# yewsiang/Transferable3D

Measured on AMD Instinct MI355X. Metric: frustums/sec fwd+bwd, higher is better.
Workload: dtype f32

## Files before the change

include/t3d.h:

```cpp
#ifndef T3D_H_
#define T3D_H_

#include <stdint.h>

#ifdef __cplusplus
extern "C" {
#endif

#define T3D_OK 0
#define T3D_ERR_ARG (-1)
#define T3D_ERR_SHAPE (-2)
#define T3D_ERR_LAUNCH (-3)
#define T3D_ERR_ABI (-4)

#define T3D_ABI_VERSION 3
#define T3D_V2_SIZE_pointmlp_fwd_args 200
#define T3D_V2_SIZE_pointmlp_dgrad_args 168
#define T3D_V2_SIZE_pointmlp_wgrad_args 144
#define T3D_V2_SIZE_pointmlp_dgrad_gram_args 168
#define T3D_V2_SIZE_pointmlp_gram_args 96
#define T3D_V2_SIZE_seg_head_args 208
#define T3D_V2_SIZE_boxpc_rep_args 104

#define T3D_TILE_ROWS 128
// ... 159 lines not shown
typedef struct {
  const float* psum_dz;
  const float* psum_y;
  const float* coef;
  int B, N, tiles_per_frustum, rows_per_frustum;
  float alpha;
  float* out;
} t3d_dy_colsum_args;
int t3d_dy_colsum(const t3d_dy_colsum_args* args, t3d_stream_t stream);

typedef struct {
  const float* w;
  const float* bias;
  const float* coef;
  int K, N;
  float* p_slabs;
  float* rc_slabs;
  float* wc;
} t3d_pool_bwd_prep_args;
int t3d_pool_bwd_prep(const t3d_pool_bwd_prep_args* args, t3d_stream_t stream);

typedef struct {
  const int32_t* argidx;
  const float* dpool;
  const float* wc;
  int B, N, K;
  int rows_per_frustum;
  float* s;
  int32_t* row_live;
} t3d_pool_sparse_rows_args;
int t3d_pool_sparse_rows(const t3d_pool_sparse_rows_args* args, t3d_stream_t stream);

typedef struct {
  uint32_t struct_size;
  t3d_act_src a;
  const float* p;
  const float* rowconst;
  const float* add_in;
  const int32_t* add_live;
  const float* prev_y;
  const float* prev_scale;
  const float* prev_shift;
  float* out;
  float* psum_dz;
  float* psum_dzy;
  int M, K;
  int rows_per_frustum;
  int dtype;
  int arith;
} t3d_pointmlp_dgrad_gram_args;
int t3d_pointmlp_dgrad_gram(const t3d_pointmlp_dgrad_gram_args* args, t3d_stream_t stream);

typedef struct {
  uint32_t struct_size;
  t3d_act_src a;
  float* slabs;
  int M, K;
  int rows_per_frustum;
  int rows_per_split;
  int arith;
} t3d_pointmlp_gram_args;
int t3d_pointmlp_gram(const t3d_pointmlp_gram_args* args, t3d_stream_t stream);

int t3d_gram_plan(int M, int K, int dtype, int* rows_per_split, int* one_pass);

typedef struct {
  t3d_act_src a;
  int M, K;
  int rows_per_frustum;
  float* part;
} t3d_act_colsum_args;
int t3d_act_colsum(const t3d_act_colsum_args* args, t3d_stream_t stream);

typedef struct {
  t3d_act_src a;
  const int32_t* argidx;
  const float* dpool;
  const float* coef;
  const float* w;
  const float* bias;
  const float* g;
  const float* abar;
  int B, K, N;
  int rows_per_frustum;
  float* dw;
} t3d_pool_wgrad_finish_args;
int t3d_pool_wgrad_finish(const t3d_pool_wgrad_finish_args* args, t3d_stream_t stream);

int t3d_pool_bwd_stage1(const t3d_pointmlp_gram_args* gram, const t3d_act_colsum_args* colsum,
                        const t3d_pool_bwd_prep_args* prep, t3d_stream_t stream);
int t3d_pool_bwd_stage2(const t3d_pool_wgrad_finish_args* finish, const t3d_pointmlp_dgrad_gram_args* dgrad,
                        t3d_stream_t stream);

typedef struct {
  const float* in;  int ld_in;  int K;
  const float* in2; int ld_in2; int K2;
  const float* w;
  const float* bias;
  const float* gamma; const float* beta;
  float* moving_mean; float* moving_var;
  const float* decay;
  float eps; int is_training; int unbiased_ema;
  int act; float leaky_alpha;
  const float* drop_mask; float keep_prob;
  const float* add_in; int ld_add; int add_n;
  float* y;
  float* out; int ld_out;
  float* mean; float* invstd;
  int B, N;
} t3d_fc_fwd_args;
int t3d_fc_fwd(const t3d_fc_fwd_args* args, t3d_stream_t stream);

typedef struct {
  const float* dout; int ld_dout;
  const float* dy_next; const float* w_next; int N_next;
  const float* in;  int ld_in;  int K;
  const float* in2; int ld_in2; int K2;
  const float* y; const float* out; int ld_out;
  const float* gamma; const float* beta; const float* mean; const float* invstd;
  int bn_training;
  int act; float leaky_alpha;
  const float* drop_mask; float keep_prob;
  float* dy;
  float* dw; float* dbias; float* dgamma; float* dbeta;
  int B, N;
// ... 410 lines not shown
  float bn_init_decay, bn_decay_rate, bn_decay_step, bn_decay_clip;
  float beta1, beta2;
  int batch_size;
  int step_offset;
} t3d_schedule;
int t3d_schedule_step(float* hyper, const t3d_schedule* s, t3d_stream_t stream);

int t3d_adam_tf_step(float* params, const float* grads, float* m, float* v, int64_t n,
                     const float* hyper, float beta1, float beta2, float eps, float grad_scale,
                     t3d_stream_t stream);

typedef struct { int64_t off; int64_t n; int32_t blk0; int32_t reserved; } t3d_adam_range;
int t3d_reduce_slabs_adam(const float* slab_base, float* grad_base, const t3d_slab_desc* table_dev, int n_tensors, int max_numel,
                          float* params, float* m, float* v, const t3d_adam_range* ranges_dev, int n_ranges, int n_range_blocks,
                          const float* hyper, float beta1, float beta2, float eps, float grad_scale, t3d_stream_t stream);

int t3d_split_x3(const float* src, void* planes, int64_t n, int64_t plane_stride, t3d_stream_t stream);

typedef struct {
  int64_t off;
  int32_t K, N;
  int32_t fwd, dgrad;
  int32_t blk0;
  int32_t reserved;
} t3d_x3_frag_entry;
int t3d_split_x3_frag(const float* params, void* planes_fwd, void* planes_dgrad, int64_t plane_stride, const t3d_x3_frag_entry* table,
                      int n_entries, int n_blocks, t3d_stream_t stream);

int t3d_step_head_takes(const t3d_pointmlp_fwd_args* fwd);
int t3d_step_head(const t3d_pointmlp_fwd_args* fwd, const float* params, void* planes_fwd, void* planes_dgrad, int64_t plane_stride,
                  const t3d_x3_frag_entry* table, int n_entries, int n_blocks, float* hyper, const t3d_schedule* sched,
                  t3d_stream_t stream);

int t3d_momentum_step(float* params, const float* grads, float* accum, int64_t n, const float* hyper, float momentum,
                      float grad_scale, t3d_stream_t stream);

typedef struct {
  t3d_act_src a;
  const float* mask;
  float keep_prob;
  float* out;
  int M, K;
  int rows_per_frustum;
} t3d_act_dropout_args;
int t3d_act_dropout(const t3d_act_dropout_args* args, t3d_stream_t stream);

int t3d_cast_bf16(const float* src, void* dst, int64_t n, t3d_stream_t stream);

int t3d_dropout_mask(float* mask, int64_t n, float keep_prob, uint32_t seed, const float* hyper,
                     t3d_stream_t stream);

enum { T3D_SMALL_BN_BWD_FINALIZE = 1, T3D_SMALL_FC_BWD = 2, T3D_SMALL_FC_DINPUT = 3, T3D_SMALL_DY_COLSUM = 4,
       T3D_SMALL_BN_FWD_FINALIZE = 5, T3D_SMALL_FC_FWD = 6, T3D_SMALL_POOL_BWD_MID = 7 };
typedef struct {
  const float* slab_base;
  float* grad_base;
  const t3d_slab_desc* table_dev;
  int n_tensors, max_numel;
  t3d_pool_sparse_rows_args sparse;
} t3d_pool_bwd_mid_args;
typedef struct {
  int kind;
  int depends;
  union {
    t3d_bn_bwd_finalize_args bn_bwd;
    t3d_fc_bwd_args fc_bwd;
    t3d_fc_dinput_args fc_dinput;
    t3d_dy_colsum_args dy_colsum;
    t3d_bn_fwd_finalize_args bn_fwd;
    t3d_fc_fwd_args fc_fwd;
    t3d_pool_bwd_mid_args mid;
  } u;
} t3d_small_op;
int t3d_small_pair(const t3d_small_op* a, const t3d_small_op* b, t3d_stream_t stream);

#define T3D_RIDER_MAX_OPS 10
typedef struct {
  t3d_small_op ops[T3D_RIDER_MAX_OPS];
  int n_ops;
  int n_wg;
  int lds_bytes;
  unsigned* sync;
} t3d_rider_set;
int t3d_riders_plan(t3d_rider_set* riders);
int t3d_run_riders(const t3d_rider_set* riders, t3d_stream_t stream);
int t3d_pointmlp_fwd_r(const t3d_pointmlp_fwd_args* args, const t3d_rider_set* riders, t3d_stream_t stream);
int t3d_pointmlp_wgrad_r(const t3d_pointmlp_wgrad_args* args, const t3d_rider_set* riders, t3d_stream_t stream);
int t3d_pointmlp_bwd_r(const t3d_pointmlp_dgrad_args* dgrad, const t3d_pointmlp_wgrad_args* wgrad, const t3d_rider_set* riders,
                       t3d_stream_t stream);
int t3d_pool_bwd_stage1_r(const t3d_pointmlp_gram_args* gram, const t3d_act_colsum_args* colsum, const t3d_pool_bwd_prep_args* prep,
                          const t3d_rider_set* riders, t3d_stream_t stream);
int t3d_pool_bwd_stage2_r(const t3d_pool_wgrad_finish_args* finish, const t3d_pointmlp_dgrad_gram_args* dgrad,
                          const t3d_rider_set* riders, t3d_stream_t stream);
int t3d_pointmlp_fwd_hosts_riders(const t3d_pointmlp_fwd_args* args);
int t3d_pointmlp_wgrad_hosts_riders(const t3d_pointmlp_wgrad_args* args);
int t3d_pointmlp_bwd_hosts_riders(const t3d_pointmlp_dgrad_args* dgrad, const t3d_pointmlp_wgrad_args* wgrad);
int t3d_pool_bwd_stage1_hosts_riders(const t3d_pointmlp_gram_args* gram, const t3d_act_colsum_args* colsum, const t3d_pool_bwd_prep_args* prep);
int t3d_pool_bwd_stage2_hosts_riders(const t3d_pool_wgrad_finish_args* finish, const t3d_pointmlp_dgrad_gram_args* dgrad);

typedef struct {
  uint32_t struct_size;
  const double* points;
  const int64_t* scene_offsets;
  const double* rtilt;
  const double* K;
  const int32_t* scene_jobs;
  int n_scenes; int max_scene_points; int C_src; int C; int n_jobs; int num_points;
  const double* box2d;
  int perturb_box2d;
  const double* perturb_draws;
  const double* box3d;
  const int32_t* job_key;
  uint32_t seed;
  const int32_t* choice;
  const int64_t* mask_offsets;
  uint64_t* masks;
  int32_t* seg_prefix;
  double* box2d_out;
  double* frustum_angle;
  int32_t* n_in_box;
  int32_t* count;
  int32_t* index;
  double* out_points;
  int32_t* label;
} t3d_frustum_extract_args;
#define T3D_V2_SIZE_frustum_extract_args 208
// ... 183 lines not shown
```

transferable3d_amd/abi.py:

```python
import ctypes as C
import os

F = C.POINTER(C.c_float)
I = C.POINTER(C.c_int32)
D = C.POINTER(C.c_double)
L = C.POINTER(C.c_int64)
i32, f32 = C.c_int, C.c_float

TILE_ROWS = 128
F32, BF16 = 0, 1
DTYPE_BY_NAME = {'f32': F32, 'bf16': BF16}
ARITH_AUTO, ARITH_FP32_MFMA, ARITH_BF16X3, ARITH_BF16 = 0, 1, 2, 3
ARITH_BY_NAME = {'auto': ARITH_AUTO, 'fp32_mfma': ARITH_FP32_MFMA, 'bf16x3': ARITH_BF16X3}
ARITH_NAMES = {ARITH_FP32_MFMA: 'fp32_mfma', ARITH_BF16X3: 'bf16x3', ARITH_BF16: 'bf16'}
ABI_VERSION = 3
ERR_ABI = -4
ACT_NONE, ACT_RELU, ACT_LEAKY_RELU, ACT_TANH = 0, 1, 2, 3
ACT_BY_NAME = {None: ACT_NONE, 'relu': ACT_RELU, 'leaky_relu': ACT_LEAKY_RELU, 'tanh': ACT_TANH}


class Sized(C.Structure):

    def __init__(self, *args, **kw):
        super().__init__(C.sizeof(type(self)), *args, **kw)
# ... 18 lines not shown
    _fields_ = [('psum', F), ('psumsq', F), ('n_tiles', i32), ('count', i32), ('N', i32), ('gamma', F), ('beta', F),
                ('moving_mean', F), ('moving_var', F), ('decay', F), ('eps', f32), ('is_training', i32),
                ('unbiased_ema', i32), ('scale', F), ('shift', F), ('mean', F), ('invstd', F),
                ('pool_pmax', F), ('pool_pmin', F), ('pool_pamax', I), ('pool_pamin', I), ('pool_B', i32), ('pool_tiles_per_frustum', i32),
                ('pooled', F), ('ld_pooled', i32), ('argidx', I), ('ysel', F)]


class PoolFinalizeArgs(C.Structure):
    _fields_ = [('scale', F), ('shift', F), ('pmax', F), ('pmin', F), ('pamax', I), ('pamin', I),
                ('B', i32), ('N', i32), ('tiles_per_frustum', i32), ('pooled', F), ('ld_pooled', i32),
                ('argidx', I), ('ysel', F)]


class PointMlpDgradArgs(Sized):
    _fields_ = [('struct_size', C.c_uint32), ('dy', DySrc), ('w', F), ('add_in', F), ('prev_y', F), ('prev_scale', F), ('prev_shift', F),
                ('out', F), ('psum_dz', F), ('psum_dzy', F), ('M', i32), ('K', i32), ('N', i32),
                ('rows_per_frustum', i32), ('dtype', i32), ('w_x3', C.c_void_p), ('w_x3_stride', C.c_int64), ('arith', i32)]


class PointMlpWgradArgs(Sized):
    _fields_ = [('struct_size', C.c_uint32), ('a', ActSrc), ('dy', DySrc), ('slabs', F), ('M', i32), ('K', i32), ('N', i32),
                ('rows_per_frustum', i32), ('rows_per_split', i32), ('arith', i32)]


class PoolBwdPrepArgs(C.Structure):
    _fields_ = [('w', F), ('bias', F), ('coef', F), ('K', i32), ('N', i32), ('p_slabs', F), ('rc_slabs', F), ('wc', F)]


class PoolSparseRowsArgs(C.Structure):
    _fields_ = [('argidx', I), ('dpool', F), ('wc', F), ('B', i32), ('N', i32), ('K', i32), ('rows_per_frustum', i32), ('s', F),
                ('row_live', I)]


class PointMlpDgradGramArgs(Sized):
    _fields_ = [('struct_size', C.c_uint32), ('a', ActSrc), ('p', F), ('rowconst', F), ('add_in', F), ('add_live', I), ('prev_y', F), ('prev_scale', F),
                ('prev_shift', F),
                ('out', F), ('psum_dz', F), ('psum_dzy', F), ('M', i32), ('K', i32), ('rows_per_frustum', i32), ('dtype', i32), ('arith', i32)]


class PointMlpGramArgs(Sized):
    _fields_ = [('struct_size', C.c_uint32), ('a', ActSrc), ('slabs', F), ('M', i32), ('K', i32), ('rows_per_frustum', i32), ('rows_per_split', i32), ('arith', i32)]


class ActColsumArgs(C.Structure):
    _fields_ = [('a', ActSrc), ('M', i32), ('K', i32), ('rows_per_frustum', i32), ('part', F)]


class PoolWgradFinishArgs(C.Structure):
    _fields_ = [('a', ActSrc), ('argidx', I), ('dpool', F), ('coef', F), ('w', F), ('bias', F), ('g', F), ('abar', F),
                ('B', i32), ('K', i32), ('N', i32), ('rows_per_frustum', i32), ('dw', F)]


class BoxRefineStepArgs(C.Structure):
    _fields_ = [('out9', F), ('center_in', F), ('dims_in', F), ('theta_in', F), ('center_out', F), ('dims_out', F), ('theta_out', F),
                ('total', F), ('fit_prob', F), ('weigh_by_conf', i32), ('first', i32), ('B', i32)]


class ClassGroups(C.Structure):
    _fields_ = [('members', I), ('offsets', I), ('n_groups', i32), ('perm', I), ('perm_len', i32)]


class SampleEqualClassesArgs(C.Structure):
    _fields_ = [('set', ClassGroups * 2), ('B', i32), ('seed', C.c_uint32), ('hyper', F), ('order_draws', F), ('member_draws', F),
                ('equal_prob', f32), ('prob_draw', F), ('sample', I), ('is_data_2D', I)]


# ... 90 lines not shown

class ActDropoutArgs(C.Structure):
    _fields_ = [('a', ActSrc), ('mask', F), ('keep_prob', f32), ('out', F), ('M', i32), ('K', i32), ('rows_per_frustum', i32)]


class SegFinalizeArgs(C.Structure):
    _fields_ = [('part', F), ('dw_part', F), ('B', i32), ('tiles_per_frustum', i32), ('rows_per_frustum', i32),
                ('K', i32), ('mask_xyz_mean', F), ('seg_loss', F), ('dw', F), ('dbias', F), ('n_correct', F)]


class StrongWeights(C.Structure):
    _fields_ = [(n, f32) for n in ('center', 'orient_cls', 'orient_reg', 'dims_cls', 'dims_reg', 'tnet_center',
                                   'corner', 'box_multiplier', 'cross_entropy')]


class StrongLossArgs(C.Structure):
    _fields_ = [('box', F), ('ld_box', i32), ('stage1_center', F), ('seg_loss', F), ('y_center', F),
                ('y_orient_cls', I), ('y_orient_reg', F), ('y_dims_cls', I), ('y_dims_reg', F), ('is_data_2D', I),
                ('wts', StrongWeights), ('normalize_by_3d_count', i32), ('dbox', F), ('dstage1', F), ('terms', F),
                ('total_losses', F), ('loss', F), ('center', F), ('reg_dims', F), ('reg_theta', F), ('iou2d', F), ('iou3d', F), ('B', i32)]


class X3FragEntry(C.Structure):
    _fields_ = [('off', C.c_int64), ('K', C.c_int32), ('N', C.c_int32), ('fwd', C.c_int32), ('dgrad', C.c_int32), ('blk0', C.c_int32), ('reserved', C.c_int32)]


def x3_frag_table(entries):
    import numpy as np
    rec = np.zeros(len(entries), dtype=np.dtype([('off', '<i8'), ('K', '<i4'), ('N', '<i4'), ('fwd', '<i4'), ('dgrad', '<i4'), ('blk0', '<i4'), ('reserved', '<i4')]))
    blk = 0
    for i, (off, K, N) in enumerate(entries):
        rec[i] = (off, K, N, 1, 1, blk, 0)
        blk += (K * N // 8 + 255) // 256
    return rec.view(np.uint8).copy(), blk


class SlabDesc(C.Structure):
    _fields_ = [('slab_off', C.c_int64), ('grad_off', C.c_int64), ('numel', C.c_int32), ('n_slabs', C.c_int32)]


class AdamRange(C.Structure):
    _fields_ = [('off', C.c_int64), ('n', C.c_int64), ('blk0', C.c_int32), ('reserved', C.c_int32)]


ADAM_RANGE_ELEMS = 1024


def adam_range_table(n_total, slab_tensors):
    out, pos, blk = [], 0, 0
    for off, n in sorted(slab_tensors):
        if n <= 0 or off < pos or off + n > n_total:
            raise T3DError('slab tensors overlap or leave the parameter buffer: (%d, %d) after %d of %d' % (off, n, pos, n_total))
        if off > pos:
            out.append((pos, off - pos, blk))
            blk += (off - pos + ADAM_RANGE_ELEMS - 1) // ADAM_RANGE_ELEMS
        pos = off + n
    if pos < n_total:
        out.append((pos, n_total - pos, blk))
        blk += (n_total - pos + ADAM_RANGE_ELEMS - 1) // ADAM_RANGE_ELEMS
    assert sum(n for _, n, _ in out) + sum(n for _, n in slab_tensors) == n_total
    return out, blk


class Schedule(C.Structure):
    _fields_ = [('base_lr', f32), ('lr_decay_rate', f32), ('lr_decay_step', f32), ('bn_init_decay', f32),
                ('bn_decay_rate', f32), ('bn_decay_step', f32), ('bn_decay_clip', f32), ('beta1', f32), ('beta2', f32),
# ... 185 lines not shown


ENTRY_POINTS = {
    't3d_abi_version': [],
    't3d_gemm_arithmetic': [i32, i32, i32, i32, i32],
    't3d_source_hash': [C.c_char_p, C.c_int],
    't3d_pointmlp_fwd': [C.POINTER(PointMlpFwdArgs), VP],
    't3d_bn_fwd_finalize': [C.POINTER(BnFwdFinalizeArgs), VP],
    't3d_pool_finalize': [C.POINTER(PoolFinalizeArgs), VP],
    't3d_pointmlp_dgrad': [C.POINTER(PointMlpDgradArgs), VP],
    't3d_pointmlp_wgrad': [C.POINTER(PointMlpWgradArgs), VP],
    't3d_pointmlp_bwd': [C.POINTER(PointMlpDgradArgs), C.POINTER(PointMlpWgradArgs), VP],
    't3d_wgrad_plan': [i32, i32, i32, C.POINTER(i32), C.POINTER(i32), C.POINTER(i32)],
    't3d_bwd_plan': [i32, i32, i32, i32, C.POINTER(i32), C.POINTER(i32)],
    't3d_weak_loss': [C.POINTER(WeakLossArgs), VP],
    't3d_small_pair': [C.POINTER(SmallOp), C.POINTER(SmallOp), VP],
    't3d_riders_plan': [C.POINTER(RiderSet)],
    't3d_run_riders': [C.POINTER(RiderSet), VP],
    't3d_pointmlp_fwd_r': [C.POINTER(PointMlpFwdArgs), C.POINTER(RiderSet), VP],
    't3d_pointmlp_wgrad_r': [C.POINTER(PointMlpWgradArgs), C.POINTER(RiderSet), VP],
    't3d_pointmlp_bwd_r': [C.POINTER(PointMlpDgradArgs), C.POINTER(PointMlpWgradArgs), C.POINTER(RiderSet), VP],
    't3d_pool_bwd_stage1_r': [C.POINTER(PointMlpGramArgs), C.POINTER(ActColsumArgs), C.POINTER(PoolBwdPrepArgs), C.POINTER(RiderSet), VP],
    't3d_pool_bwd_stage2_r': [C.POINTER(PoolWgradFinishArgs), C.POINTER(PointMlpDgradGramArgs), C.POINTER(RiderSet), VP],
    't3d_pointmlp_fwd_hosts_riders': [C.POINTER(PointMlpFwdArgs)],
    't3d_pointmlp_wgrad_hosts_riders': [C.POINTER(PointMlpWgradArgs)],
    't3d_pointmlp_bwd_hosts_riders': [C.POINTER(PointMlpDgradArgs), C.POINTER(PointMlpWgradArgs)],
    't3d_pool_bwd_stage1_hosts_riders': [C.POINTER(PointMlpGramArgs), C.POINTER(ActColsumArgs), C.POINTER(PoolBwdPrepArgs)],
    't3d_pool_bwd_stage2_hosts_riders': [C.POINTER(PoolWgradFinishArgs), C.POINTER(PointMlpDgradGramArgs)],
    't3d_gram_plan': [i32, i32, i32, C.POINTER(i32), C.POINTER(i32)],
    't3d_bn_bwd_finalize': [C.POINTER(BnBwdFinalizeArgs), VP],
    't3d_dy_colsum': [C.POINTER(DyColsumArgs), VP],
    't3d_pool_bwd_prep': [C.POINTER(PoolBwdPrepArgs), VP],
    't3d_pool_sparse_rows': [C.POINTER(PoolSparseRowsArgs), VP],
    't3d_pointmlp_dgrad_gram': [C.POINTER(PointMlpDgradGramArgs), VP],
    't3d_pointmlp_gram': [C.POINTER(PointMlpGramArgs), VP],
    't3d_act_colsum': [C.POINTER(ActColsumArgs), VP],
    't3d_pool_wgrad_finish': [C.POINTER(PoolWgradFinishArgs), VP],
    't3d_batch_assemble': [C.POINTER(BatchAssembleArgs), VP],
    't3d_box_refine_step': [C.POINTER(BoxRefineStepArgs), VP],
    't3d_box_refine_step_bwd': [C.POINTER(BoxRefineStepBwdArgs), VP],
    't3d_boxpc_perturb': [C.POINTER(BoxPcPerturbArgs), VP],
    't3d_sample_equal_classes': [C.POINTER(SampleEqualClassesArgs), VP],
    't3d_box3d_iou': [C.POINTER(Box3dIouArgs), VP],
    't3d_box3d_iou_corners': [C.POINTER(Box3dIouCornersArgs), VP],
    't3d_box_head_iou': [C.POINTER(BoxHeadIouArgs), VP],
    't3d_box2d_feats': [C.POINTER(Box2dFeatsArgs), VP],
    't3d_pool_bwd_stage1': [C.POINTER(PointMlpGramArgs), C.POINTER(ActColsumArgs), C.POINTER(PoolBwdPrepArgs), VP],
    't3d_pool_bwd_mid': [F, F, C.POINTER(SlabDesc), i32, i32, C.POINTER(PoolSparseRowsArgs), VP],
    't3d_pool_bwd_stage2': [C.POINTER(PoolWgradFinishArgs), C.POINTER(PointMlpDgradGramArgs), VP],
    't3d_fc_fwd': [C.POINTER(FcFwdArgs), VP],
    't3d_fc_bwd': [C.POINTER(FcBwdArgs), VP],
    't3d_fc_dinput': [C.POINTER(FcDinputArgs), VP],
    't3d_seg_head': [C.POINTER(SegHeadArgs), VP],
    't3d_seg_finalize': [C.POINTER(SegFinalizeArgs), VP],
    't3d_act_dropout': [C.POINTER(ActDropoutArgs), VP],
    't3d_strong_loss': [C.POINTER(StrongLossArgs), VP],
    't3d_boxpc_rep': [C.POINTER(BoxPcRepArgs), VP],
    't3d_boxpc_rep_b': [C.POINTER(BoxPcRepBArgs), VP],
    't3d_boxpc_rep_bwd': [C.POINTER(BoxPcRepBwdArgs), VP],
    't3d_boxpc_loss': [C.POINTER(BoxPcLossArgs), VP],
    't3d_pointmlp_dgrad_narrow': [C.POINTER(DgradNarrowArgs), VP],
    't3d_semi_final_loss': [C.POINTER(SemiFinalLossArgs), VP],
    't3d_anchor_reg_bwd': [C.POINTER(AnchorRegBwdArgs), VP],
    't3d_reduce_slabs': [F, F, C.POINTER(SlabDesc), i32, i32, VP],
    't3d_schedule_step': [F, C.POINTER(Schedule), VP],
    't3d_reduce_slabs_adam': [F, F, C.POINTER(SlabDesc), i32, i32, F, F, F, C.POINTER(AdamRange), i32, i32, F, f32, f32, f32, f32, VP],
    't3d_step_head_takes': [C.POINTER(PointMlpFwdArgs)],
    't3d_step_head': [C.POINTER(PointMlpFwdArgs), F, VP, VP, C.c_int64, VP, i32, i32, F, C.POINTER(Schedule), VP],
    't3d_adam_tf_step': [F, F, F, F, C.c_int64, F, f32, f32, f32, f32, VP],
    't3d_momentum_step': [F, F, F, C.c_int64, F, f32, f32, VP],
    't3d_split_x3': [F, VP, C.c_int64, C.c_int64, VP],
    't3d_split_x3_frag': [F, VP, VP, C.c_int64, VP, i32, i32, VP],
    't3d_dropout_mask': [F, C.c_int64, f32, C.c_uint32, F, VP],
    't3d_cast_bf16': [F, VP, C.c_int64, VP],
    't3d_frustum_extract': [C.POINTER(FrustumExtractArgs), VP],
    't3d_sunrgbd_eval': [C.POINTER(SunrgbdEvalArgs), VP],
    't3d_sunrgbd_diagnose': [C.POINTER(SunrgbdEvalArgs), C.POINTER(SunrgbdDiagnoseArgs), VP],
    't3d_detect_decode': [C.POINTER(DetectDecodeArgs), VP],
    't3d_detect_nms': [C.POINTER(DetectNmsArgs), VP],
    't3d_render': [C.POINTER(RenderArgs), VP],
    't3d_semi_sample': [C.POINTER(SemiSampleArgs), VP],
    't3d_label_subset': [C.POINTER(LabelSubsetArgs), VP],
}

LIB_PATH = os.path.join(os.path.dirname(os.path.abspath(__file__)), 'libt3d.so')
ERRORS = {-1: 'T3D_ERR_ARG', -2: 'T3D_ERR_SHAPE', -3: 'T3D_ERR_LAUNCH'}


class T3DError(RuntimeError):
    pass


def source_hash_of(lib):
    buf = C.create_string_buffer(64)
    check(lib.t3d_source_hash(buf, 64), 't3d_source_hash')
    return buf.value.decode()


def load(path=None):
    import torch
    variant = path or os.environ.get('T3D_LIB')
# ... 37 lines not shown
```

transferable3d_amd/csrc/bn_optim.hip:

```cpp
#include "common.h"
#include "poolbwd_dev.h"
#include "bn_dev.h"

namespace {

template <int GR, int CH = FC_CH>
__global__ __launch_bounds__(GR * CH) void k_bn_fwd_finalize(const t3d_bn_fwd_finalize_args p) {
  __shared__ double red[GR][CH];
  __shared__ float s_scsh[2 * CH];
  bn_fwd_finalize_body<GR, CH>(p, red, s_scsh, blockIdx.x);
}

__global__ __launch_bounds__(256) void k_pool_finalize(const t3d_pool_finalize_args p) {
  const int i = blockIdx.x * blockDim.x + threadIdx.x;
  if (i >= p.B * p.N) return;
  const int b = i / p.N, c = i % p.N;
  pool_pick_impl(p.pmax, p.pmin, p.pamax, p.pamin, p.tiles_per_frustum, p.N, b, c, p.scale[c], p.shift[c], p.pooled, p.ld_pooled,
                 p.argidx, p.ysel);
}

template <int GR, int CH = FC_CH>
__global__ __launch_bounds__(GR * CH) void k_bn_bwd_finalize(const t3d_bn_bwd_finalize_args p) {
  __shared__ double red[GR][CH];
  bn_bwd_finalize_body<GR, CH>(p, red, blockIdx.x, threadIdx.x);
// ... 225 lines not shown
    if (i + 8 <= n) {
      const float4 a = *reinterpret_cast<const float4*>(src + i), b = *reinterpret_cast<const float4*>(src + i + 4);
      const bf16x8 h = {(bf16_t)a.x, (bf16_t)a.y, (bf16_t)a.z, (bf16_t)a.w, (bf16_t)b.x, (bf16_t)b.y, (bf16_t)b.z, (bf16_t)b.w};
      *reinterpret_cast<bf16x8*>(dst + i) = h;
    } else {
      for (int64_t j = i; j < n; ++j) dst[j] = (bf16_t)src[j];
    }
  }
}

extern "C" int t3d_cast_bf16(const float* src, void* dst, int64_t n, t3d_stream_t stream) {
  if (!src || !dst || n <= 0 || (reinterpret_cast<uintptr_t>(src) & 15) || (reinterpret_cast<uintptr_t>(dst) & 15)) return T3D_ERR_ARG;
  int64_t blocks = (n + 2047) / 2048;
  if (blocks > 2048) blocks = 2048;
  T3D_LAUNCH(k_cast_bf16, dim3((unsigned)blocks), dim3(256), 0, static_cast<hipStream_t>(stream), src, static_cast<bf16_t*>(dst), n);
  T3D_CHECK_LAUNCH();
  return T3D_OK;
}

extern "C" int t3d_dropout_mask(float* mask, int64_t n, float keep_prob, uint32_t seed, const float* hyper,
                                t3d_stream_t stream) {
  if (!mask || !hyper || n <= 0) return T3D_ERR_ARG;
  int64_t blocks = (n + 255) / 256;
  if (blocks > 4096) blocks = 4096;
  T3D_LAUNCH(k_dropout_mask, dim3((unsigned)blocks), dim3(256), 0, static_cast<hipStream_t>(stream), mask, n,
                     keep_prob, seed, hyper);
  T3D_CHECK_LAUNCH();
  return T3D_OK;
}

extern "C" int t3d_pool_bwd_mid(const float* slab_base, float* grad_base, const t3d_slab_desc* table_dev, int n_tensors,
                                int max_numel, const t3d_pool_sparse_rows_args* a, t3d_stream_t stream) {
  if (!slab_base || !grad_base || !table_dev || n_tensors <= 0) return T3D_ERR_ARG;
  const int rc = check_sparse_rows(a);
  if (rc != T3D_OK) return rc;
  int gx = (max_numel / 4 + 31) / 32;
  if (gx > 256) gx = 256;
  if (gx < 1) gx = 1;
  const int n_reduce = gx * n_tensors;
  const long M = (long)a->B * a->rows_per_frustum;
  const int n_sparse = (int)(M / 128) * (a->K / SR_KC);
  const size_t lds = sparse_rows_lds(a->N);
  static size_t allowed = 0;
  if (lds > 64 * 1024 && lds > allowed) {
    (void)hipFuncSetAttribute(reinterpret_cast<const void*>(k_pool_bwd_mid), hipFuncAttributeMaxDynamicSharedMemorySize, (int)lds);
    allowed = lds;
  }
  T3D_LAUNCH(k_pool_bwd_mid, dim3(n_reduce + n_sparse), dim3(256), lds, static_cast<hipStream_t>(stream), slab_base, grad_base,
             table_dev, gx, n_reduce, *a);
  T3D_CHECK_LAUNCH();
  return T3D_OK;
}
```

transferable3d_amd/csrc/pointmlp.hip:

```cpp
#include "common.h"
#include "poolbwd_dev.h"
#include "rider_dev.h"

#include <cstdlib>
#include <mutex>
#include <type_traits>
#include <utility>
#include <unordered_map>

namespace {

constexpr int BK = 32;
constexpr int MIN_WAVES_PER_EU = 2;
constexpr int LDR = BK + 4;
constexpr int NT = 256;

__device__ __forceinline__ float4 f4zero() { return make_float4(0.f, 0.f, 0.f, 0.f); }

__device__ __forceinline__ unsigned keep_bits32(const float* __restrict__ rowmask, int base) {
  float4 m[8];
#pragma unroll
  for (int q = 0; q < 8; ++q) m[q] = *reinterpret_cast<const float4*>(rowmask + base + (q >> 2) * 32 + (q & 3) * 8);
  unsigned bits = 0u;
#pragma unroll
// ... 2830 lines not shown
}

template <int BN, class PR = PathF32>
__global__ __launch_bounds__(NT, MIN_WAVES_PER_EU) void k_pool_bwd_stage2(const t3d_pool_wgrad_finish_args f,
                                                                   const t3d_pointmlp_dgrad_gram_args d, const int n_finish) {
  extern __shared__ __attribute__((aligned(16))) float smem[];
  const int b = blockIdx.x;
  if (b < n_finish) {
    const int kb = f.K / FK;
    pool_wgrad_finish_body<typename PR::T>(f, smem, b % kb, b / kb);
  } else {
    dgrad_gram_body<BN, PR>(d, smem, b - n_finish, gridDim.x - n_finish);
  }
}

template <int GT, class PR = PathF32>
__global__ __launch_bounds__(NT, MIN_WAVES_PER_EU) void k_pool_bwd_stage1_r(const t3d_pointmlp_gram_args g, const t3d_act_colsum_args c,
                                                                     const t3d_pool_bwd_prep_args q, const int n_gram,
                                                                     const int n_colsum, const t3d_rider_set r) {
  extern __shared__ __attribute__((aligned(16))) float smem[];
  if ((int)blockIdx.x < r.n_wg) { run_riders(r, smem); return; }
  const int b = blockIdx.x - r.n_wg;
  if (b < n_gram) {
    typename PR::template Act<false, float> la{g.a, g.K, g.rows_per_frustum};
    wgrad_body<GT, GT, PR, true>(la, la, g.slabs, g.K, g.K, g.rows_per_split, smem, b, n_gram);
  } else if (b < n_gram + n_colsum) {
    act_colsum_body<float>(c, smem, b - n_gram);
  } else {
    const int rr = b - n_gram - n_colsum, kb = q.K / 32;
    pool_bwd_prep_body(q, smem, rr % kb, (rr / kb) % kb, rr / (kb * kb));
  }
}

template <int BN, class PR = PathF32>
__global__ __launch_bounds__(NT, MIN_WAVES_PER_EU) void k_pool_bwd_stage2_r(const t3d_pool_wgrad_finish_args f,
                                                                     const t3d_pointmlp_dgrad_gram_args d, const int n_finish,
                                                                     const t3d_rider_set r) {
  extern __shared__ __attribute__((aligned(16))) float smem[];
  if ((int)blockIdx.x < r.n_wg) { run_riders(r, smem); return; }
  const int b = blockIdx.x - r.n_wg;
  if (b < n_finish) {
    const int kb = f.K / FK;
    pool_wgrad_finish_body<float>(f, smem, b % kb, b / kb);
  } else {
    dgrad_gram_body<BN, PR>(d, smem, b - n_finish, (int)gridDim.x - r.n_wg - n_finish);
  }
}

template <int K, int BM>
__device__ __forceinline__ void gram1_body(const t3d_pointmlp_gram_args& g, float* part, float* smem, int split) {
  constexpr int CPA = K / 8, RPA = NT1 / CPA, NIA = BM / RPA;
  constexpr int KT = K / 32, TMW = KT / 2, TNW = KT / 4;
  bf16_t* Aimg = reinterpret_cast<bf16_t*>(smem);
  float* csum = reinterpret_cast<float*>(Aimg + 2 * BM * K);
  const int tid = threadIdx.x, lane = tid & 63, wv = tid >> 6, l31 = lane & 31, h = lane >> 5;
  const int kt0 = (wv >> 2) * TMW, nt0 = (wv & 3) * TNW;
  const int cha = tid % CPA, ra = tid / CPA;
  const int row_begin = split * g.rows_per_split, n_tiles = g.rows_per_split / BM;
  const bf16_t* xg = reinterpret_cast<const bf16_t*>(g.a.x);
  const float floor_ = g.a.relu ? 0.f : -INFINITY;

  bf16x8 rx[NIA];
  auto load_raw = [&](int row0) {
#pragma unroll
    for (int i = 0; i < NIA; ++i)
      rx[i] = *reinterpret_cast<const bf16x8*>(xg + (size_t)(row0 + ra + RPA * i) * g.a.ldx + g.a.coff + cha * 8);
// ... 537 lines not shown
  if (arith == T3D_ARITH_FP32_MFMA) return false;
  if (arith == T3D_ARITH_BF16X3) return true;
  const char* e = getenv("T3D_X3");
  return e ? atoi(e) != 0 : true;
}
long x3_min_kn(int arith) { const char* e = arith == T3D_ARITH_AUTO ? getenv("T3D_X3_MINKN") : nullptr; return e ? atol(e) : 1L; }
long x3_min_kn_bwd(int arith) { const char* e = arith == T3D_ARITH_AUTO ? getenv("T3D_X3_MINKN_BWD") : nullptr; return e ? atol(e) : x3_min_kn(arith); }
bool x3_layer(int arith, int K, int N) { return x3_on(arith) && (long)K * N >= x3_min_kn(arith) && K <= 4096 && N <= 4096; }
bool x3_bwd_narrow() { const char* e = getenv("T3D_X3_BWD_NARROW"); return e ? atoi(e) != 0 : true; }
bool x3_layer_bwd(int arith, int K, int N) {
  return x3_on(arith) && (long)K * N >= x3_min_kn_bwd(arith) && (N <= 4 * K || K >= 128 || x3_bwd_narrow()) && K <= 4096 && N <= 4096;
}
bool act_ok(const t3d_act_src& a, int K) {
  return a.x != nullptr && (a.ldx % 4) == 0 && (a.coff % 4) == 0 && a.coff + (K + 3) / 4 * 4 <= a.ldx &&
         (a.scale == nullptr || a.shift != nullptr) && dtype_ok(a.dtype) && !(a.dtype == T3D_BF16 && a.sub != nullptr) &&
         !(a.dtype == T3D_BF16 && ((a.ldx | a.coff) & 7));
}
bool dy_ok(const t3d_dy_src& d) {
  return d.y != nullptr && d.coef != nullptr && (d.dz != nullptr || (d.argidx != nullptr && d.dpool != nullptr)) && dtype_ok(d.dtype) &&
         !(d.dtype == T3D_BF16 && d.dz == nullptr);
}

bool riders_ok(const t3d_rider_set* r) {
  return r->sync != nullptr && r->n_ops > 0 && r->n_ops <= T3D_RIDER_MAX_OPS && r->n_wg > 0 && r->n_wg <= (r->n_ops == 1 ? RIDER_MAX_WG_WIDE : RIDER_MAX_WG) && r->lds_bytes >= 0;
}
size_t lds_with(size_t lds, const t3d_rider_set* r) { return r && (size_t)r->lds_bytes > lds ? (size_t)r->lds_bytes : lds; }

}

int t3d_x3_fwd(const t3d_pointmlp_fwd_args* a, const t3d_rider_set* r, hipStream_t s);
int t3d_x3_bwd(const t3d_pointmlp_dgrad_args* d, const t3d_pointmlp_wgrad_args* w, const t3d_rider_set* r, int tk, int tn, bool wide,
               int n_w, int n_d, hipStream_t s);
int t3d_x3_stage1(const t3d_pointmlp_gram_args* g, const t3d_act_colsum_args* c, const t3d_pool_bwd_prep_args* q, const t3d_rider_set* r,
                  int gt, int n_gram, int n_colsum, int n_prep, size_t lds_other, hipStream_t s);
int t3d_x3_stage2(const t3d_pool_wgrad_finish_args* f, const t3d_pointmlp_dgrad_gram_args* d, const t3d_rider_set* r, bool wide,
                  int n_finish, int n_d, size_t lds_other, hipStream_t s);
int t3d_x3_split(const float* src, void* planes, int64_t n, int64_t plane_stride, hipStream_t s);
int t3d_x3_split_frag(const float* params, void* pf, void* pd, int64_t stride, const t3d_x3_frag_entry* tab, int n, int n_blocks, hipStream_t s);
int t3d_x3_step_head(const t3d_pointmlp_fwd_args* a, const float* params, void* pf, void* pd, int64_t stride, const t3d_x3_frag_entry* tab, int n,
                     int n_blocks, float* hyper, const t3d_schedule* sched, hipStream_t s);
int t3d_x3_dgrad(const t3d_pointmlp_dgrad_args* a, bool wide, hipStream_t s);
int t3d_x3_wgrad(const t3d_pointmlp_wgrad_args* a, int tk, int tn, int n_blocks, hipStream_t s);
int t3d_x3_gram(const t3d_pointmlp_gram_args* a, int tk, int n_blocks, hipStream_t s);
int t3d_x3_dgrad_gram(const t3d_pointmlp_dgrad_gram_args* a, bool wide, hipStream_t s);

#ifdef T3D_X3_TU
namespace {
__global__ __launch_bounds__(256) void k_split_x3(const float* __restrict__ src, bf16_t* __restrict__ planes, long n, long stride) {
  const long step = (long)gridDim.x * 256 * 4;
  for (long i = ((long)blockIdx.x * 256 + threadIdx.x) * 4; i < n; i += step) {
    if (i + 4 <= n) {
      bf16x4 h, m, l;
      split3(*reinterpret_cast<const float4*>(src + i), h, m, l);
      *reinterpret_cast<bf16x4*>(planes + i) = h;
      *reinterpret_cast<bf16x4*>(planes + stride + i) = m;
      *reinterpret_cast<bf16x4*>(planes + 2 * stride + i) = l;
    } else {
      for (long j = i; j < n; ++j) {
        bf16x4 h, m, l;
        split3(make_float4(src[j], 0.f, 0.f, 0.f), h, m, l);
        planes[j] = h[0]; planes[stride + j] = m[0]; planes[2 * stride + j] = l[0];
      }
    }
  }
}
}
namespace {
__device__ __forceinline__ void split_x3_frag_body(const float* __restrict__ params, bf16_t* __restrict__ pf, bf16_t* __restrict__ pd, long stride,
                                                   const t3d_x3_frag_entry* __restrict__ tab, int n, const int blk) {
  int e = 0;
  while (e + 1 < n && blk >= tab[e + 1].blk0) ++e;
  const t3d_x3_frag_entry en = tab[e];
  const float* w = params + en.off;
// ... 5 lines not shown
  float4 v0, v1, u0, u1;
  if (en.fwd) {
    const int NB = en.N / 32, nb = (int)(q % NB);
    const long k0 = (q / NB) * 16 + 8 * (lane >> 5);
    const float* src = w + k0 * en.N + nb * 32 + (lane & 31);
    v0 = make_float4(src[0], src[en.N], src[2 * (long)en.N], src[3 * (long)en.N]);
    v1 = make_float4(src[4 * (long)en.N], src[5 * (long)en.N], src[6 * (long)en.N], src[7 * (long)en.N]);
  }
  if (en.dgrad) {
    const int KB = en.K / 32, kb = (int)(q % KB);
    const long n0 = (q / KB) * 16 + 8 * (lane >> 5);
    const float* src = w + (long)(kb * 32 + (lane & 31)) * en.N + n0;
    u0 = *reinterpret_cast<const float4*>(src);
    u1 = *reinterpret_cast<const float4*>(src + 4);
  }
  bf16x4 h0, m0, l0, h1, m1, l1;
  if (en.fwd) {
    split3(v0, h0, m0, l0);
    split3(v1, h1, m1, l1);
    bf16_t* d = pf + en.off + f * 8;
    *reinterpret_cast<bf16x8*>(d) = __builtin_shufflevector(h0, h1, 0, 1, 2, 3, 4, 5, 6, 7);
    *reinterpret_cast<bf16x8*>(d + stride) = __builtin_shufflevector(m0, m1, 0, 1, 2, 3, 4, 5, 6, 7);
    *reinterpret_cast<bf16x8*>(d + 2 * stride) = __builtin_shufflevector(l0, l1, 0, 1, 2, 3, 4, 5, 6, 7);
  }
  if (en.dgrad) {
    split3(u0, h0, m0, l0);
    split3(u1, h1, m1, l1);
    bf16_t* d = pd + en.off + f * 8;
    *reinterpret_cast<bf16x8*>(d) = __builtin_shufflevector(h0, h1, 0, 1, 2, 3, 4, 5, 6, 7);
    *reinterpret_cast<bf16x8*>(d + stride) = __builtin_shufflevector(m0, m1, 0, 1, 2, 3, 4, 5, 6, 7);
    *reinterpret_cast<bf16x8*>(d + 2 * stride) = __builtin_shufflevector(l0, l1, 0, 1, 2, 3, 4, 5, 6, 7);
  }
}
__global__ __launch_bounds__(256) void k_split_x3_frag(const float* __restrict__ params, bf16_t* __restrict__ pf, bf16_t* __restrict__ pd, long stride,
                                                       const t3d_x3_frag_entry* __restrict__ tab, int n) {
  split_x3_frag_body(params, pf, pd, stride, tab, n, (int)blockIdx.x);
}

template <int N>
__global__ __launch_bounds__(NT) void k_step_head(const t3d_pointmlp_fwd_args p, const int n_fwd, const float* __restrict__ params,
                                                  bf16_t* __restrict__ pf, bf16_t* __restrict__ pd, const long stride,
                                                  const t3d_x3_frag_entry* __restrict__ tab, const int n, const int n_split, float* hyper,
                                                  const t3d_schedule sched) {
  __shared__ float red[2][NT / (N / 8)][N];
  const int b = blockIdx.x;
  if (b < n_fwd) pointmlp_fwd_tinyk_body<N, float>(p, red, b);
  else if (b < n_fwd + n_split) split_x3_frag_body(params, pf, pd, stride, tab, n, b - n_fwd);
  else if (threadIdx.x < 64) schedule_step_body(hyper, sched, threadIdx.x);
}
}
int t3d_x3_step_head(const t3d_pointmlp_fwd_args* a, const float* params, void* pf, void* pd, int64_t stride, const t3d_x3_frag_entry* tab, int n,
                     int n_blocks, float* hyper, const t3d_schedule* sched, hipStream_t s) {
  static_assert(NT == 256, "the three roles of k_step_head are 256-thread workgroups");
  const int n_fwd = a->M / 128;
  const dim3 grid(n_fwd + n_blocks + 1);
  if (a->N == 64) T3D_LAUNCH(k_step_head<64>, grid, dim3(NT), 0, s, *a, n_fwd, params, static_cast<bf16_t*>(pf), static_cast<bf16_t*>(pd), (long)stride, tab, n, n_blocks, hyper, *sched);
  else T3D_LAUNCH(k_step_head<128>, grid, dim3(NT), 0, s, *a, n_fwd, params, static_cast<bf16_t*>(pf), static_cast<bf16_t*>(pd), (long)stride, tab, n, n_blocks, hyper, *sched);
  T3D_CHECK_LAUNCH();
  return T3D_OK;
}
int t3d_x3_split_frag(const float* params, void* pf, void* pd, int64_t stride, const t3d_x3_frag_entry* tab, int n, int n_blocks, hipStream_t s) {
  T3D_LAUNCH(k_split_x3_frag, dim3(n_blocks), dim3(256), 0, s, params, static_cast<bf16_t*>(pf), static_cast<bf16_t*>(pd), (long)stride, tab, n);
  T3D_CHECK_LAUNCH();
  return T3D_OK;
}
int t3d_x3_split(const float* src, void* planes, int64_t n, int64_t plane_stride, hipStream_t s) {
  long blocks = (n + 1023) / 1024;
  if (blocks > 2048) blocks = 2048;
  T3D_LAUNCH(k_split_x3, dim3((unsigned)blocks), dim3(256), 0, s, src, static_cast<bf16_t*>(planes), (long)n, (long)plane_stride);
  T3D_CHECK_LAUNCH();
  return T3D_OK;
}

int t3d_x3_dgrad(const t3d_pointmlp_dgrad_args* a, bool wide, hipStream_t s) {
  const int tiles_m = a->M / 128;
  if (a->w_x3 && (a->K % 32 != 0 || a->N % 16 != 0 || a->w_x3_stride < (int64_t)a->K * a->N)) return T3D_ERR_SHAPE;
  if (a->w_x3 && a->N <= X3_CTAB_MAX_CH) {
    if (wide) launch_lds(k_pointmlp_dgrad<128, false, PathX3P>, dim3(tiles_m * (a->K / 128)), lds_dgrad_x3(128), s, *a);
    else launch_lds(k_pointmlp_dgrad<64, false, PathX3P>, dim3(tiles_m * (a->K / 64)), lds_dgrad_x3(64), s, *a);
  } else if (wide) launch_lds(k_pointmlp_dgrad<128, false, PathX3>, dim3(tiles_m * (a->K / 128)), lds_dgrad_x3(128), s, *a);
  else launch_lds(k_pointmlp_dgrad<64, false, PathX3>, dim3(tiles_m * (a->K / 64)), lds_dgrad_x3(64), s, *a);
  T3D_CHECK_LAUNCH();
  return T3D_OK;
}

int t3d_x3_wgrad(const t3d_pointmlp_wgrad_args* a, int tk, int tn, int n_blocks, hipStream_t s) {
  const dim3 grid(n_blocks);
#define T3D_WGX(TK, TN_) launch_lds(k_pointmlp_wgrad<TK, TN_, false, false, PathX3, float>, grid, lds_wgrad_x3(TK, TN_), s, *a)
  if (tk == 128 && tn == 128) T3D_WGX(128, 128);
  else if (tk == 128) T3D_WGX(128, 64);
  else if (tn == 128) T3D_WGX(64, 128);
  else T3D_WGX(64, 64);
#undef T3D_WGX
  T3D_CHECK_LAUNCH();
  return T3D_OK;
// ... 65 lines not shown
  if (d->w_x3 && (d->K % 32 != 0 || d->N % 16 != 0 || d->w_x3_stride < (int64_t)d->K * d->N)) return T3D_ERR_SHAPE;
  const dim3 grid(n_w + n_d + (r ? r->n_wg : 0));
#define T3D_BWDX_P(DBN, TK, TN_, PR_)                                                             \
  do {                                                                                             \
    const size_t lds = lds_max(lds_dgrad_x3(DBN), lds_wgrad_x3(TK, TN_));                          \
    if (r) {                                                                                       \
      auto kern = k_pointmlp_bwd_r<DBN, TK, TN_, PR_>;                                             \
      allow_lds(reinterpret_cast<const void*>(kern), lds_with(lds, r));                            \
      T3D_LAUNCH(kern, grid, dim3(NT), lds_with(lds, r), s, *d, *w, n_w, *r);                      \
    } else {                                                                                       \
      auto kern = k_pointmlp_bwd<DBN, TK, TN_, PR_>;                                               \
      allow_lds(reinterpret_cast<const void*>(kern), lds);                                         \
      T3D_LAUNCH(kern, grid, dim3(NT), lds, s, *d, *w, n_w);                                       \
    }                                                                                              \
  } while (0)
#define T3D_BWDX(DBN, TK, TN_) do { if (d->w_x3 && d->N <= X3_CTAB_MAX_CH) T3D_BWDX_P(DBN, TK, TN_, PathX3P); else T3D_BWDX_P(DBN, TK, TN_, PathX3); } while (0)
#define T3D_BWDX_W(DBN)                                  \
  do {                                                   \
    if (tk == 128 && tn == 128) T3D_BWDX(DBN, 128, 128); \
    else if (tk == 128) T3D_BWDX(DBN, 128, 64);          \
    else if (tn == 128) T3D_BWDX(DBN, 64, 128);          \
    else T3D_BWDX(DBN, 64, 64);                          \
  } while (0)
  if (wide) T3D_BWDX_W(128);
  else T3D_BWDX_W(64);
#undef T3D_BWDX_W
#undef T3D_BWDX
#undef T3D_BWDX_P
  T3D_CHECK_LAUNCH();
  return T3D_OK;
}

int t3d_x3_stage1(const t3d_pointmlp_gram_args* g, const t3d_act_colsum_args* c, const t3d_pool_bwd_prep_args* q, const t3d_rider_set* r,
                  int gt, int n_gram, int n_colsum, int n_prep, size_t lds_other, hipStream_t s) {
  const dim3 grid(n_gram + n_colsum + n_prep + (r ? r->n_wg : 0));
  const size_t lds = lds_with(lds_max(lds_wgrad_x3(gt, gt), lds_other), r);
#define T3D_ST1X(GT_)                                                                  \
  do {                                                                                 \
    if (r) {                                                                           \
      auto kern = k_pool_bwd_stage1_r<GT_, PathX3>;                                    \
      allow_lds(reinterpret_cast<const void*>(kern), lds);                             \
      T3D_LAUNCH(kern, grid, dim3(NT), lds, s, *g, *c, *q, n_gram, n_colsum, *r);      \
    } else {                                                                           \
      auto kern = k_pool_bwd_stage1<GT_, PathX3>;                                      \
      allow_lds(reinterpret_cast<const void*>(kern), lds);                             \
      T3D_LAUNCH(kern, grid, dim3(NT), lds, s, *g, *c, *q, n_gram, n_colsum);          \
    }                                                                                  \
  } while (0)
  if (gt != 64) return T3D_ERR_ARG;
  T3D_ST1X(64);
#undef T3D_ST1X
  T3D_CHECK_LAUNCH();
  return T3D_OK;
}

int t3d_x3_stage2(const t3d_pool_wgrad_finish_args* f, const t3d_pointmlp_dgrad_gram_args* d, const t3d_rider_set* r, bool wide,
                  int n_finish, int n_d, size_t lds_other, hipStream_t s) {
  const dim3 grid(n_finish + n_d + (r ? r->n_wg : 0));
  const size_t lds = lds_with(lds_max(wide ? lds_fwd_x3(128) : lds_fwd_x3(64), lds_other), r);
#define T3D_ST2X(BN_)                                                                  \
  do {                                                                                 \
    if (r) {                                                                           \
      auto kern = k_pool_bwd_stage2_r<BN_, PathX3>;                                    \
      allow_lds(reinterpret_cast<const void*>(kern), lds);                             \
      T3D_LAUNCH(kern, grid, dim3(NT), lds, s, *f, *d, n_finish, *r);                  \
    } else {                                                                           \
      auto kern = k_pool_bwd_stage2<BN_, PathX3>;                                      \
// ... 516 lines not shown
  do {                                                                                                              \
    if (bf16) {                                                                                                     \
      const size_t lds = lds_dgrad_h(DBN) > lds_wgrad_h(TK, TN_) ? lds_dgrad_h(DBN) : lds_wgrad_h(TK, TN_);         \
      auto kern = k_pointmlp_bwd<DBN, TK, TN_, PathBF16>;                                                           \
      allow_lds(reinterpret_cast<const void*>(kern), lds);                                                          \
      T3D_LAUNCH(kern, grid, dim3(NT), lds, s, *d, *w, n_w);                                                        \
    } else if (r) {                                                                                                 \
      const size_t lds = lds_with(lds_dgrad(DBN) > lds_wgrad(TK, TN_) ? lds_dgrad(DBN) : lds_wgrad(TK, TN_), r);    \
      auto kern = k_pointmlp_bwd_r<DBN, TK, TN_>;                                                                   \
      allow_lds(reinterpret_cast<const void*>(kern), lds);                                                          \
      T3D_LAUNCH(kern, grid, dim3(NT), lds, s, *d, *w, n_w, *r);                                                    \
    } else {                                                                                                        \
      const size_t lds = lds_dgrad(DBN) > lds_wgrad(TK, TN_) ? lds_dgrad(DBN) : lds_wgrad(TK, TN_);                 \
      auto kern = k_pointmlp_bwd<DBN, TK, TN_>;                                                                     \
      allow_lds(reinterpret_cast<const void*>(kern), lds);                                                          \
      T3D_LAUNCH(kern, grid, dim3(NT), lds, s, *d, *w, n_w);                                                        \
    }                                                                                                               \
  } while (0)
#define T3D_BWD_W(DBN)                              \
  do {                                              \
    if (tk == 128 && tn == 128) T3D_BWD(DBN, 128, 128); \
    else if (tk == 128) T3D_BWD(DBN, 128, 64);      \
    else if (tn == 128) T3D_BWD(DBN, 64, 128);      \
    else T3D_BWD(DBN, 64, 64);                      \
  } while (0)
  if (wide) T3D_BWD_W(128);
  else T3D_BWD_W(64);
#undef T3D_BWD_W
#undef T3D_BWD
  T3D_CHECK_LAUNCH();
  return T3D_OK;
}

extern "C" int t3d_pool_bwd_stage1(const t3d_pointmlp_gram_args* g, const t3d_act_colsum_args* c,
                                   const t3d_pool_bwd_prep_args* q, t3d_stream_t stream) {
  return t3d_pool_bwd_stage1_r(g, c, q, nullptr, stream);
}

extern "C" int t3d_pool_bwd_stage1_r(const t3d_pointmlp_gram_args* g, const t3d_act_colsum_args* c,
                                     const t3d_pool_bwd_prep_args* q, const t3d_rider_set* r, t3d_stream_t stream) {
  T3D_ABI_TAKE(pointmlp_gram_args, g);
  if (r && !riders_ok(r)) return T3D_ERR_ARG;
  int rc = check_gram(g);
  if (rc != T3D_OK) return rc;
  if ((rc = check_colsum(c)) != T3D_OK) return rc;
  if ((rc = check_prep(q)) != T3D_OK) return rc;
  hipStream_t s = static_cast<hipStream_t>(stream);
  if (c->a.dtype != g->a.dtype) return T3D_ERR_ARG;
  if (gram1_ok(g) && c->M == g->M && c->K == g->K && c->a.x == g->a.x && c->a.ldx == g->a.ldx && c->a.coff == g->a.coff) {
    T3D_RIDERS_FIRST(r, stream);
    const int n_gram1 = g->M / g->rows_per_split, n_prep1 = (q->K / 32) * (q->K / 32) * ((q->N + PCH - 1) / PCH);
    const dim3 grid1(n_gram1 + (n_prep1 + 1) / 2);
#define T3D_ST1H(K_, BM_)                                                                                  \
  do {                                                                                                     \
    const size_t lds1 = lds_max(lds_gram1(K_, BM_), 2 * PREP_LDS);                                         \
    auto kern = k_pool_bwd_stage1_h<K_, BM_>;                                                              \
    allow_lds(reinterpret_cast<const void*>(kern), lds1);                                                  \
    T3D_LAUNCH(kern, grid1, dim3(NT1), lds1, s, *g, *c, *q, n_gram1);                                      \
  } while (0)
    if (g->K == 128) T3D_ST1H(128, 128); else T3D_ST1H(256, 64);
#undef T3D_ST1H
    T3D_CHECK_LAUNCH();
    return T3D_OK;
  }
  const bool x3g = g->a.dtype != T3D_BF16 && x3_layer_bwd(g->arith, g->K, g->K);
  const int gt = x3g ? 64 : gram_tile(g);
  const int n_gram = (g->K / gt) * (g->K / gt) * (g->M / g->rows_per_split);
  const int n_colsum = c->M / 128;
  const int n_prep = (q->K / 32) * (q->K / 32) * ((q->N + PCH - 1) / PCH);
  const bool bf16 = g->a.dtype == T3D_BF16;
  if (c->a.dtype != g->a.dtype) return T3D_ERR_ARG;
  if (bf16) { T3D_RIDERS_FIRST(r, stream); r = nullptr; }
  const dim3 grid(n_gram + n_colsum + n_prep + (r ? r->n_wg : 0));
  size_t lds = bf16 ? lds_wgrad_h(gt, gt) : lds_wgrad(gt, gt);
  if (PREP_LDS > lds) lds = PREP_LDS;
  if (COLSUM_LDS > lds) lds = COLSUM_LDS;
  T3D_HOSTED(r, stream);
  if (x3g) return t3d_x3_stage1(g, c, q, r, gt, n_gram, n_colsum, n_prep, lds_max(PREP_LDS, COLSUM_LDS), s);
  lds = lds_with(lds, r);
#define T3D_ST1(GT_, PR_)                                                              \
  do {                                                                                 \
    auto kern = k_pool_bwd_stage1<GT_, PR_>;                                           \
    allow_lds(reinterpret_cast<const void*>(kern), lds);                               \
    T3D_LAUNCH(kern, grid, dim3(NT), lds, s, *g, *c, *q, n_gram, n_colsum);            \
  } while (0)
#define T3D_ST1R(GT_)                                                                  \
  do {                                                                                 \
    auto kern = k_pool_bwd_stage1_r<GT_>;                                              \
    allow_lds(reinterpret_cast<const void*>(kern), lds);                               \
    T3D_LAUNCH(kern, grid, dim3(NT), lds, s, *g, *c, *q, n_gram, n_colsum, *r);        \
  } while (0)
  if (r) { if (gt == 128) T3D_ST1R(128); else T3D_ST1R(64); }
  else if (bf16) { if (gt == 128) T3D_ST1(128, PathBF16); else T3D_ST1(64, PathBF16); }
  else { if (gt == 128) T3D_ST1(128, PathF32); else T3D_ST1(64, PathF32); }
#undef T3D_ST1R
#undef T3D_ST1
  T3D_CHECK_LAUNCH();
  return T3D_OK;
}

extern "C" int t3d_pool_bwd_stage2(const t3d_pool_wgrad_finish_args* f, const t3d_pointmlp_dgrad_gram_args* d,
                                   t3d_stream_t stream) {
  return t3d_pool_bwd_stage2_r(f, d, nullptr, stream);
}

extern "C" int t3d_pool_bwd_stage2_r(const t3d_pool_wgrad_finish_args* f, const t3d_pointmlp_dgrad_gram_args* d,
                                     const t3d_rider_set* r, t3d_stream_t stream) {
  T3D_ABI_TAKE(pointmlp_dgrad_gram_args, d);
  if (r && !riders_ok(r)) return T3D_ERR_ARG;
  int rc = check_finish(f);
  if (rc != T3D_OK) return rc;
// ... 32 lines not shown
#define T3D_ST2(BN_, PR_)                                                              \
  do {                                                                                 \
    auto kern = k_pool_bwd_stage2<BN_, PR_>;                                           \
    allow_lds(reinterpret_cast<const void*>(kern), lds);                               \
    T3D_LAUNCH(kern, grid, dim3(NT), lds, s, *f, *d, n_finish);                        \
  } while (0)
#define T3D_ST2R(BN_)                                                                  \
  do {                                                                                 \
    auto kern = k_pool_bwd_stage2_r<BN_>;                                              \
    allow_lds(reinterpret_cast<const void*>(kern), lds);                               \
    T3D_LAUNCH(kern, grid, dim3(NT), lds, s, *f, *d, n_finish, *r);                    \
  } while (0)
  if (r) { if (wide) T3D_ST2R(128); else T3D_ST2R(64); }
  else if (bf16) { if (wide) T3D_ST2(128, PathBF16); else T3D_ST2(64, PathBF16); }
  else { if (wide) T3D_ST2(128, PathF32); else T3D_ST2(64, PathF32); }
#undef T3D_ST2R
#undef T3D_ST2
  T3D_CHECK_LAUNCH();
  return T3D_OK;
}

extern "C" int t3d_split_x3(const float* src, void* planes, int64_t n, int64_t plane_stride, t3d_stream_t stream) {
  if (!src || !planes || n <= 0 || plane_stride < n || (reinterpret_cast<uintptr_t>(src) & 15) || (reinterpret_cast<uintptr_t>(planes) & 7) ||
      (plane_stride & 3))
    return T3D_ERR_ARG;
  return t3d_x3_split(src, planes, n, plane_stride, static_cast<hipStream_t>(stream));
}

extern "C" int t3d_split_x3_frag(const float* params, void* planes_fwd, void* planes_dgrad, int64_t plane_stride, const t3d_x3_frag_entry* table,
                                 int n_entries, int n_blocks, t3d_stream_t stream) {
  if (!params || !planes_fwd || !planes_dgrad || !table || n_entries <= 0 || n_blocks <= 0 || plane_stride <= 0 || (plane_stride & 7) ||
      (reinterpret_cast<uintptr_t>(params) & 15) || (reinterpret_cast<uintptr_t>(planes_fwd) & 15) || (reinterpret_cast<uintptr_t>(planes_dgrad) & 15))
    return T3D_ERR_ARG;
  return t3d_x3_split_frag(params, planes_fwd, planes_dgrad, plane_stride, table, n_entries, n_blocks, static_cast<hipStream_t>(stream));
}

static int step_head_fwd_check(const t3d_pointmlp_fwd_args* a) {
  if (!a || !a->w || !a->psum || !a->psumsq || !act_ok(a->a, a->K)) return T3D_ERR_ARG;
  if (a->M <= 0 || a->K <= 0 || a->N <= 0 || a->M % T3D_TILE_ROWS || a->rows_per_frustum % T3D_TILE_ROWS ||
      a->M % a->rows_per_frustum || a->N % 64 || (long)a->M * a->N >= (1L << 30))
    return T3D_ERR_SHAPE;
  if (a->dtype != T3D_F32 || a->a.dtype != T3D_F32 || !fwd_takes_tinyk32(a) || a->a.scale || a->a.shift || a->a.sub) return T3D_ERR_ARG;
  return T3D_OK;
}

extern "C" int t3d_step_head_takes(const t3d_pointmlp_fwd_args* a) {
  T3D_ABI_TAKE(pointmlp_fwd_args, a);
  return step_head_fwd_check(a) == T3D_OK ? 1 : 0;
}

extern "C" int t3d_step_head(const t3d_pointmlp_fwd_args* a, const float* params, void* planes_fwd, void* planes_dgrad, int64_t plane_stride,
                             const t3d_x3_frag_entry* table, int n_entries, int n_blocks, float* hyper, const t3d_schedule* sched,
                             t3d_stream_t stream) {
  T3D_ABI_TAKE(pointmlp_fwd_args, a);
  if (!hyper || !sched) return T3D_ERR_ARG;
  if (!params || !planes_fwd || !planes_dgrad || !table || n_entries <= 0 || n_blocks <= 0 || plane_stride <= 0 || (plane_stride & 7) ||
      (reinterpret_cast<uintptr_t>(params) & 15) || (reinterpret_cast<uintptr_t>(planes_fwd) & 15) || (reinterpret_cast<uintptr_t>(planes_dgrad) & 15))
    return T3D_ERR_ARG;
  const int rc = step_head_fwd_check(a);
  if (rc != T3D_OK) return rc;
  return t3d_x3_step_head(a, params, planes_fwd, planes_dgrad, plane_stride, table, n_entries, n_blocks, hyper, sched, static_cast<hipStream_t>(stream));
}

static const t3d_rider_set* query_set() {
  static const t3d_rider_set q = []() { t3d_rider_set r{}; r.n_ops = 1; r.n_wg = 1; r.sync = reinterpret_cast<unsigned*>(16); return r; }();
  return &q;
}
extern "C" int t3d_gemm_arithmetic(int arith, int dtype, int K, int N, int kind) {
  if (dtype == T3D_BF16) return T3D_ARITH_BF16;
  bool x3 = false;
  switch (kind) {
    case T3D_GEMM_FWD: x3 = K % BKX == 0 && x3_layer(arith, K, N); break;
    case T3D_GEMM_BWD: x3 = N % BKX == 0 && K % 64 == 0 && (K <= 64 || K % 128 == 0) && x3_layer_bwd(arith, K, N); break;
    case T3D_GEMM_DGRAD: x3 = N % BKX == 0 && x3_layer_bwd(arith, K, N); break;
    case T3D_GEMM_WGRAD: x3 = K % 64 == 0 && (K <= 64 || K % 128 == 0) && x3_layer_bwd(arith, K, N); break;
    case T3D_GEMM_GRAM: x3 = x3_layer_bwd(arith, K, K); break;
    case T3D_GEMM_DGRAD_GRAM: x3 = K % BKX == 0 && x3_layer_bwd(arith, K, K); break;
    default: return T3D_ERR_ARG;
  }
  return x3 ? T3D_ARITH_BF16X3 : T3D_ARITH_FP32_MFMA;
}
extern "C" int t3d_pointmlp_fwd_hosts_riders(const t3d_pointmlp_fwd_args* a) { return t3d_pointmlp_fwd_r(a, query_set(), T3D_QUERY_STREAM); }
extern "C" int t3d_pointmlp_wgrad_hosts_riders(const t3d_pointmlp_wgrad_args* a) { return t3d_pointmlp_wgrad_r(a, query_set(), T3D_QUERY_STREAM); }
extern "C" int t3d_pointmlp_bwd_hosts_riders(const t3d_pointmlp_dgrad_args* d, const t3d_pointmlp_wgrad_args* w) {
  return t3d_pointmlp_bwd_r(d, w, query_set(), T3D_QUERY_STREAM);
}
extern "C" int t3d_pool_bwd_stage1_hosts_riders(const t3d_pointmlp_gram_args* g, const t3d_act_colsum_args* c, const t3d_pool_bwd_prep_args* q) {
  return t3d_pool_bwd_stage1_r(g, c, q, query_set(), T3D_QUERY_STREAM);
}
extern "C" int t3d_pool_bwd_stage2_hosts_riders(const t3d_pool_wgrad_finish_args* f, const t3d_pointmlp_dgrad_gram_args* d) {
  return t3d_pool_bwd_stage2_r(f, d, query_set(), T3D_QUERY_STREAM);
}

#ifdef T3D_TRACE
// ... 16 lines not shown
```

transferable3d_amd/csrc/poolbwd.hip:

```cpp
#include "poolbwd_dev.h"

namespace {

__global__ __launch_bounds__(256) void k_pool_bwd_prep(const t3d_pool_bwd_prep_args p) {
  extern __shared__ __attribute__((aligned(16))) float smem[];
  pool_bwd_prep_body(p, smem, blockIdx.x, blockIdx.y, blockIdx.z);
}
__global__ __launch_bounds__(256) void k_pool_sparse_rows(const t3d_pool_sparse_rows_args p) {
  extern __shared__ __attribute__((aligned(16))) float smem[];
  pool_sparse_rows_body(p, smem, blockIdx.x, blockIdx.y);
}
template <class XT>
__global__ __launch_bounds__(256) void k_act_colsum(const t3d_act_colsum_args p) {
  extern __shared__ __attribute__((aligned(16))) float smem[];
  act_colsum_body<XT>(p, smem, blockIdx.x);
}
template <class XT>
__global__ __launch_bounds__(256) void k_pool_wgrad_finish(const t3d_pool_wgrad_finish_args p) {
  extern __shared__ __attribute__((aligned(16))) float smem[];
  pool_wgrad_finish_body<XT>(p, smem, blockIdx.x, blockIdx.y);
}

}

extern "C" int t3d_pool_bwd_prep(const t3d_pool_bwd_prep_args* a, t3d_stream_t stream) {
  const int rc = check_prep(a);
  if (rc != T3D_OK) return rc;
  T3D_LAUNCH(k_pool_bwd_prep, dim3(a->K / 32, a->K / 32, (a->N + PCH - 1) / PCH), dim3(256), PREP_LDS,
             static_cast<hipStream_t>(stream), *a);
  T3D_CHECK_LAUNCH();
  return T3D_OK;
}

extern "C" int t3d_pool_sparse_rows(const t3d_pool_sparse_rows_args* a, t3d_stream_t stream) {
  const int rc = check_sparse_rows(a);
  if (rc != T3D_OK) return rc;
  const size_t lds = sparse_rows_lds(a->N);
  static size_t allowed = 0;
  if (lds > 64 * 1024 && lds > allowed) {
    (void)hipFuncSetAttribute(reinterpret_cast<const void*>(k_pool_sparse_rows), hipFuncAttributeMaxDynamicSharedMemorySize,
                              (int)lds);
    allowed = lds;
  }
  const long M = (long)a->B * a->rows_per_frustum;
  T3D_LAUNCH(k_pool_sparse_rows, dim3(M / 128, a->K / SR_KC), dim3(256), lds, static_cast<hipStream_t>(stream), *a);
  T3D_CHECK_LAUNCH();
  return T3D_OK;
}

extern "C" int t3d_act_colsum(const t3d_act_colsum_args* a, t3d_stream_t stream) {
  const int rc = check_colsum(a);
  if (rc != T3D_OK) return rc;
  if (a->a.dtype == T3D_BF16) T3D_LAUNCH(k_act_colsum<bf16_t>, dim3(a->M / 128), dim3(256), COLSUM_LDS, static_cast<hipStream_t>(stream), *a);
  else T3D_LAUNCH(k_act_colsum<float>, dim3(a->M / 128), dim3(256), COLSUM_LDS, static_cast<hipStream_t>(stream), *a);
  T3D_CHECK_LAUNCH();
  return T3D_OK;
}

extern "C" int t3d_pool_wgrad_finish(const t3d_pool_wgrad_finish_args* a, t3d_stream_t stream) {
  const int rc = check_finish(a);
  if (rc != T3D_OK) return rc;
  const size_t lds = finish_lds(a->K);
  if (a->a.dtype == T3D_BF16) T3D_LAUNCH(k_pool_wgrad_finish<bf16_t>, dim3(a->K / FK, a->N / FN), dim3(256), lds, static_cast<hipStream_t>(stream), *a);
  else T3D_LAUNCH(k_pool_wgrad_finish<float>, dim3(a->K / FK, a->N / FN), dim3(256), lds, static_cast<hipStream_t>(stream), *a);
  T3D_CHECK_LAUNCH();
  return T3D_OK;
}
```

transferable3d_amd/csrc/poolbwd_dev.h:

```cpp
#pragma once
#include "common.h"

namespace {


constexpr int PCH = 128;

constexpr size_t PREP_LDS = (2 * 32 * (PCH + 1) + 2 * PCH) * sizeof(float);

__device__ __forceinline__ void pool_bwd_prep_body(const t3d_pool_bwd_prep_args& p, float* smem, int bi, int bj, int ch, int tid_ = -1) {
  float (*wi)[PCH + 1] = reinterpret_cast<float (*)[PCH + 1]>(smem);
  float (*wj)[PCH + 1] = reinterpret_cast<float (*)[PCH + 1]>(smem + 32 * (PCH + 1));
  float* v = smem + 2 * 32 * (PCH + 1);
  float* c0s = v + PCH;
  const int tid = tid_ < 0 ? (int)threadIdx.x : tid_, ti = tid >> 4, tj = tid & 15;
  const int n0 = ch * PCH;
  const bool edge = bj == 0;
  const float* c0 = p.coef;
  const float* c1 = p.coef + p.N;
  const float* c2 = p.coef + 2 * p.N;
#pragma unroll
  for (int q = 0; q < 4; ++q) {
    const int f = tid + 256 * q;
    const int r = f >> 5, c = (f & 31) * 4;
// ... 68 lines not shown
      const int n = nb + 64 * q + lane;
      const int r = rr[q] - rin0;
      const bool hit = n < p.N && r >= 0 && r < 128 && (r & 3) == w;
      const unsigned long long m = __ballot(hit);
      if (hit) mine[cnt + __popcll(m & ((1ull << lane) - 1ull))] = n | (r << 16);
      cnt += __popcll(m);
    }
  }
  __syncthreads();
  for (int i0 = 0; i0 < cnt; i0 += SR_UNROLL) {
    float2 wv[SR_UNROLL];
    float g[SR_UNROLL];
    int rr[SR_UNROLL], en[SR_UNROLL];
#pragma unroll
    for (int u = 0; u < SR_UNROLL; ++u) en[u] = mine[min(i0 + u, cnt - 1)];
#pragma unroll
    for (int u = 0; u < SR_UNROLL; ++u) {
      const int n = en[u] & 0xffff;
      rr[u] = en[u] >> 16;
      g[u] = p.dpool[(size_t)b * p.N + n];
      wv[u] = *reinterpret_cast<const float2*>(p.wc + (size_t)n * p.K + kc0 + 2 * lane);
    }
#pragma unroll
    for (int u = 0; u < SR_UNROLL; ++u) {
      hitrow[rr[u]] = 1;
      g[u] = (i0 + u < cnt) ? g[u] : 0.f;
    }
#pragma unroll
    for (int u = 0; u < SR_UNROLL; ++u) {
      float2* t = reinterpret_cast<float2*>(tile + rr[u] * SR_KC + 2 * lane);
      float2 cur = *t;
      cur.x = fmaf(g[u], wv[u].x, cur.x);
      cur.y = fmaf(g[u], wv[u].y, cur.y);
      *t = cur;
    }
  }
  __syncthreads();
  const bool gated = p.row_live != nullptr;
  if (gated && by == 0 && tid < 128) p.row_live[row0 + tid] = hitrow[tid];
  for (int f = tid; f < 128 * SR_KC / 4; f += 256) {
    const int r = f / (SR_KC / 4), c4 = f % (SR_KC / 4);
    if (gated && !hitrow[r]) continue;
    *reinterpret_cast<float4*>(p.s + (size_t)(row0 + r) * p.K + kc0 + 4 * c4) = reinterpret_cast<const float4*>(tile)[f];
  }
}

__device__ __forceinline__ float act_elem(const t3d_act_src& s, size_t row, int k) {
  float v = ld_elem(s.x, row * s.ldx + s.coff + k, s.dtype);
  if (s.scale) v = fmaf(v, s.scale[k], s.shift[k]);
  if (s.relu) v = fmaxf(v, 0.f);
  return v;
}

constexpr size_t COLSUM_LDS = 256 * sizeof(float4);

template <class XT = float>
__device__ __forceinline__ void act_colsum_body(const t3d_act_colsum_args& p, float* smem, int bx) {
  float4* red = reinterpret_cast<float4*>(smem);
  const int tid = threadIdx.x;
  const int row0 = bx * 128;
  const int chunks = p.K / 4, c4 = tid % chunks, grp = tid / chunks, groups = 256 / chunks, rows = 128 / groups;
  float4 sc = make_float4(1.f, 1.f, 1.f, 1.f), sh = make_float4(0.f, 0.f, 0.f, 0.f);
  if (p.a.scale) {
    sc = *reinterpret_cast<const float4*>(p.a.scale + 4 * c4);
    sh = *reinterpret_cast<const float4*>(p.a.shift + 4 * c4);
  }
// ... 85 lines not shown
  float a0 = 0.f, a1 = 0.f;
#pragma unroll 8
  for (int j = 0; j < p.K; ++j) {
    const float wv = wsm[j * FN + tj];
    a0 = fmaf(gsm[ti * ldg + j], wv, a0);
    a1 = fmaf(gsm[(ti + 16) * ldg + j], wv, a1);
  }
  const int n = n0 + tj;
  const float c0 = p.coef[n], c1 = p.coef[p.N + n], c2 = p.coef[2 * p.N + n];
  const float bias = p.bias ? p.bias[n] : 0.f;
  const float ab0 = p.abar[k0 + ti], ab1 = p.abar[k0 + ti + 16];
  p.dw[(size_t)(k0 + ti) * p.N + n] = fmaf(c0, gat[ti * (FN + 1) + tj], fmaf(c1, fmaf(ab0, bias, a0), ab0 * c2));
  p.dw[(size_t)(k0 + ti + 16) * p.N + n] = fmaf(c0, gat[(ti + 16) * (FN + 1) + tj], fmaf(c1, fmaf(ab1, bias, a1), ab1 * c2));
}



inline bool pool_act_ok(const t3d_act_src& a, int K) {
  return a.x != nullptr && a.coff + K <= a.ldx && (a.scale == nullptr || a.shift != nullptr) && a.sub == nullptr;
}
inline int check_prep(const t3d_pool_bwd_prep_args* a) {
  if (!a || !a->w || !a->coef || !a->p_slabs || !a->rc_slabs) return T3D_ERR_ARG;
  if (a->K <= 0 || a->K % 32 || a->N <= 0 || a->N % 4) return T3D_ERR_SHAPE;
  return T3D_OK;
}
inline size_t sparse_rows_lds(int N) { return (size_t)128 * SR_KC * sizeof(float) + ((size_t)4 * N + 128) * sizeof(int); }
inline int check_sparse_rows(const t3d_pool_sparse_rows_args* a) {
  if (!a || !a->argidx || !a->dpool || !a->wc || !a->s) return T3D_ERR_ARG;
  if (a->B <= 0 || a->N <= 0 || a->N > 65535 || a->K % SR_KC || a->rows_per_frustum % T3D_TILE_ROWS ||
      a->rows_per_frustum > 32767 || sparse_rows_lds(a->N) > 160 * 1024)
    return T3D_ERR_SHAPE;
  return T3D_OK;
}
inline int check_colsum(const t3d_act_colsum_args* a) {
  if (!a || !a->part || !pool_act_ok(a->a, a->K)) return T3D_ERR_ARG;
  if (a->M <= 0 || a->M % T3D_TILE_ROWS || (a->K != 64 && a->K != 128 && a->K != 256) || a->a.ldx % 4 || a->a.coff % 4)
    return T3D_ERR_SHAPE;
  return T3D_OK;
}
inline int check_finish(const t3d_pool_wgrad_finish_args* a) {
  if (!a || !a->argidx || !a->dpool || !a->coef || !a->w || !a->g || !a->abar || !a->dw || !pool_act_ok(a->a, a->K))
    return T3D_ERR_ARG;
  if (a->K <= 0 || a->K % FK || a->K > 256 || a->N <= 0 || a->N % FN || a->B <= 0) return T3D_ERR_SHAPE;
  return T3D_OK;
}

}
```

transferable3d_amd/csrc/rider_dev.h:

```cpp
#pragma once
#include "fc_dev.h"
#include "bn_dev.h"
#include "poolbwd_dev.h"

namespace {

constexpr int RIDER_NWP = 4;
constexpr int RIDER_NT = RIDER_NWP * 64;
constexpr int RIDER_MAX_WG = 32;
constexpr int RIDER_MAX_WG_WIDE = 2048;
constexpr unsigned RIDER_SPIN_LIMIT = 1u << 22;

typedef __attribute__((address_space(1))) unsigned rider_gu32;

__device__ __forceinline__ void rider_barrier(unsigned* sync, int i, int n_wg, int n_ops) {
  asm volatile("s_waitcnt vmcnt(0)" ::: "memory");
  __syncthreads();
  if (threadIdx.x == 0) {
    rider_gu32* cnt = (rider_gu32*)(sync + 2 * i);
    rider_gu32* gen = cnt + 1;
    const unsigned g0 = __hip_atomic_load(gen, __ATOMIC_RELAXED, __HIP_MEMORY_SCOPE_AGENT);
    __builtin_amdgcn_fence(__ATOMIC_RELEASE, "agent");
    asm volatile("s_waitcnt vmcnt(0)" ::: "memory");
    const unsigned old = __hip_atomic_fetch_add(cnt, 1u, __ATOMIC_RELAXED, __HIP_MEMORY_SCOPE_AGENT);
    if (old + 1u == (unsigned)n_wg) {
      __hip_atomic_store(cnt, 0u, __ATOMIC_RELAXED, __HIP_MEMORY_SCOPE_AGENT);
      asm volatile("s_waitcnt vmcnt(0)" ::: "memory");
      __hip_atomic_fetch_add(gen, 1u, __ATOMIC_RELAXED, __HIP_MEMORY_SCOPE_AGENT);
    } else {
      unsigned spins = 0;
      while (__hip_atomic_load(gen, __ATOMIC_RELAXED, __HIP_MEMORY_SCOPE_AGENT) == g0) {
        __builtin_amdgcn_s_sleep(8);
        if (++spins > RIDER_SPIN_LIMIT) {
          __hip_atomic_store((rider_gu32*)(sync + 2 * T3D_RIDER_MAX_OPS), 1u, __ATOMIC_RELAXED, __HIP_MEMORY_SCOPE_AGENT);
          break;
        }
      }
    }
    __builtin_amdgcn_fence(__ATOMIC_ACQUIRE, "agent");
    asm volatile("s_waitcnt vmcnt(0)" ::: "memory");
  }
  __syncthreads();
}

__host__ __device__ __forceinline__ int mid_gx(int max_numel) {
  int gx = (max_numel / 4 + 31) / 32;
  return gx > 256 ? 256 : (gx < 1 ? 1 : gx);
}
__host__ __device__ __forceinline__ int mid_sparse_blocks(const t3d_pool_sparse_rows_args& sp) {
  return (int)(((long)sp.B * sp.rows_per_frustum) / 128) * (sp.K / SR_KC);
}

__device__ __forceinline__ int rider_blocks(const t3d_small_op& o, int kind) {
  switch (kind) {
    case T3D_SMALL_BN_BWD_FINALIZE: return (o.u.bn_bwd.N + FC_CH - 1) / FC_CH;
    case T3D_SMALL_BN_FWD_FINALIZE: return (o.u.bn_fwd.N + FC_CH - 1) / FC_CH;
    case T3D_SMALL_FC_FWD: return (o.u.fc_fwd.N + CB - 1) / CB;
    case T3D_SMALL_FC_BWD: return (o.u.fc_bwd.N + CB - 1) / CB;
    case T3D_SMALL_FC_DINPUT: return (o.u.fc_dinput.K + CB - 1) / CB;
    case T3D_SMALL_DY_COLSUM: return (o.u.dy_colsum.B * o.u.dy_colsum.N + 255) / 256;
    case T3D_SMALL_POOL_BWD_MID: return mid_gx(o.u.mid.max_numel) * o.u.mid.n_tensors + mid_sparse_blocks(o.u.mid.sparse);
    default: return 0;
  }
}

__device__ __forceinline__ void run_riders(const t3d_rider_set& r, float* smem) {
  const int wg = blockIdx.x;
  double (*red)[FC_CH] = reinterpret_cast<double (*)[FC_CH]>(smem);
  float* scsh = smem + 2 * FC_GR * FC_CH;
  __builtin_amdgcn_s_setprio(3);
  for (int i = 0; i < r.n_ops; ++i) {
    const t3d_small_op& o = r.ops[i];
    const int kind = o.kind;
    if (i > 0) {
      if (o.depends) rider_barrier(r.sync, i, r.n_wg, r.n_ops);
      else __syncthreads();
    }
    const int nb = rider_blocks(o, kind);
    for (int b = wg; b < nb; b += r.n_wg) {
      switch (kind) {
        case T3D_SMALL_BN_BWD_FINALIZE: bn_bwd_finalize_body<FC_GR>(o.u.bn_bwd, red, b, threadIdx.x); break;
        case T3D_SMALL_BN_FWD_FINALIZE: bn_fwd_finalize_body<FC_GR>(o.u.bn_fwd, red, scsh, b); break;
// ... 2 lines not shown
        case T3D_SMALL_FC_DINPUT: fc_dinput_body<1, RIDER_NWP>(o.u.fc_dinput, smem, b); break;
        case T3D_SMALL_DY_COLSUM: dy_colsum_body(o.u.dy_colsum, b, threadIdx.x); break;
        case T3D_SMALL_POOL_BWD_MID: {
          const t3d_pool_bwd_mid_args& m = o.u.mid;
          const int gx = mid_gx(m.max_numel), n_reduce = gx * m.n_tensors;
          if (b < n_reduce) {
            reduce_slabs_body(m.slab_base, m.grad_base, m.table_dev, reinterpret_cast<float4(*)[32]>(smem), b % gx, b / gx, gx);
          } else {
            const int rr = b - n_reduce, tiles = m.sparse.B * m.sparse.rows_per_frustum / 128;
            pool_sparse_rows_body(m.sparse, smem, rr % tiles, rr / tiles);
          }
        } break;
        default: break;
      }
      __syncthreads();
    }
  }
}

inline int rider_op_blocks(const t3d_small_op& o) {
  switch (o.kind) {
    case T3D_SMALL_BN_BWD_FINALIZE:
      if (!o.u.bn_bwd.coef || (o.u.bn_bwd.psum_dz != nullptr && o.u.bn_bwd.n_tiles > 512)) return -1;
      return (o.u.bn_bwd.N + FC_CH - 1) / FC_CH;
    case T3D_SMALL_BN_FWD_FINALIZE:
      if (o.u.bn_fwd.n_tiles > 512) return -1;
      return (o.u.bn_fwd.N + FC_CH - 1) / FC_CH;
    case T3D_SMALL_FC_FWD: return o.u.fc_fwd.B <= 32 ? (o.u.fc_fwd.N + CB - 1) / CB : -1;
    case T3D_SMALL_FC_BWD: return o.u.fc_bwd.B <= 32 ? (o.u.fc_bwd.N + CB - 1) / CB : -1;
    case T3D_SMALL_FC_DINPUT: return o.u.fc_dinput.B <= 32 ? (o.u.fc_dinput.K + CB - 1) / CB : -1;
    case T3D_SMALL_DY_COLSUM: return (o.u.dy_colsum.B * o.u.dy_colsum.N + 255) / 256;
    case T3D_SMALL_POOL_BWD_MID: {
      const t3d_pool_bwd_mid_args& m = o.u.mid;
      if (!m.slab_base || !m.grad_base || !m.table_dev || m.n_tensors <= 0 || check_sparse_rows(&m.sparse) != T3D_OK) return -1;
      if (sparse_rows_lds(m.sparse.N) > 76 * 1024) return -1;
      return mid_gx(m.max_numel) * m.n_tensors + mid_sparse_blocks(m.sparse);
    }
    default: return -1;
  }
}

inline size_t rider_op_lds(const t3d_small_op& o) {
  if (o.kind == T3D_SMALL_POOL_BWD_MID) return sparse_rows_lds(o.u.mid.sparse.N);
  return fc_lds_bytes(32);
}

}
```

transferable3d_amd/engine.py:

```python
import contextlib
import ctypes as C
import math
import os

import numpy as np
import torch

from . import abi
from .abi import fptr, iptr
from .constants import BN_EPS

TILE = abi.TILE_ROWS


class Runtime:

    def __init__(self, device=None, lib=None, gemm_arithmetic=None):
        self.lib = lib if lib is not None else abi.load()
        if gemm_arithmetic is None:
            gemm_arithmetic = 'fp32_mfma' if os.environ.get('T3D_X3', '1') == '0' else 'bf16x3'
        self.gemm_arithmetic = gemm_arithmetic
        self.arith = abi.ARITH_BY_NAME[gemm_arithmetic]
        if device is None:
            if not torch.cuda.is_available():
# ... 182 lines not shown
            self.params_x3 = self.rt.zeros(3 * self.params.numel(), dtype=torch.bfloat16)
        return self.params_x3

    def x3_ptr(self, w):
        off = (w.data_ptr() - self.params.data_ptr()) // 4
        if not (0 <= off and off + w.numel() <= self.params.numel() and w.is_contiguous()) or off % 4:
            return None, 0
        return self.enable_x3().data_ptr() + 2 * off, self.params.numel()

    def x3_frag(self, w, K, N):
        off = (w.data_ptr() - self.params.data_ptr()) // 4
        none = ((None, 0), (None, 0))
        if not (0 <= off and off + w.numel() <= self.params.numel() and w.is_contiguous()) or off % 8 or K % 32 or N % 32 or w.numel() != K * N:
            return none
        n = self.params.numel()
        stride = (n + 7) // 8 * 8
        if getattr(self, 'x3_frag_planes', None) is None:
            self.x3_frag_planes = (self.rt.zeros(3 * stride, dtype=torch.bfloat16), self.rt.zeros(3 * stride, dtype=torch.bfloat16))
            self.x3_frag_entries, self.x3_frag_stride, self.x3_frag_table = {}, stride, None
        self.x3_frag_entries[off] = (K, N)
        self.x3_frag_table = None
        pf, pd = self.x3_frag_planes
        return (pf.data_ptr() + 2 * off, stride), (pd.data_ptr() + 2 * off, stride)

    def frag_table(self):
        ent = getattr(self, 'x3_frag_entries', None)
        if not ent:
            return None
        if self.x3_frag_table is None:
            raw, blocks = abi.x3_frag_table([(off, K, N) for off, (K, N) in sorted(ent.items())])
            self.x3_frag_table = (torch.from_numpy(raw).to(self.rt.device), len(ent), blocks)
        return self.x3_frag_table

    def bf16_view(self, w):
        off = (w.data_ptr() - self.params.data_ptr()) // 4
        assert 0 <= off and off + w.numel() <= self.params.numel() and w.is_contiguous()
        return self.enable_bf16()[off:off + w.numel()].view(*w.shape)

    def get(self, name):
        off, shape, trainable = self.index[name]
        buf = self.params if trainable else self.state
        return buf[off:off + int(np.prod(shape))].view(*shape)

    def grad(self, name):
        off, shape, trainable = self.index[name]
        assert trainable
        return self.grads[off:off + int(np.prod(shape))].view(*shape)

    def offset(self, name):
        return self.index[name][0]

    def xavier(self, name, shape, fan_in, fan_out):
        if name in self.index:
            return self.get(name)
        lim = math.sqrt(6.0 / (fan_in + fan_out))
        return self._alloc(name, shape, True, self.rng.uniform(-lim, lim, size=shape))

    def const(self, name, shape, val, trainable=True):
        return self._alloc(name, shape, trainable, np.full(shape, val, np.float32))

    def state_dict(self):
        return {k: self.get(k).detach().cpu().numpy().copy() for k in self.index}

    def load_state_dict(self, sd, strict=True):
        for k, v in sd.items():
            if k not in self.index:
# ... 44 lines not shown
        self.table = torch.as_tensor(raw).to(self.rt.device)
        return self


class ActSpec:

    def __init__(self, x, ldx, K, coff=0, scale=None, shift=None, relu=False, sub=None, sub_ld=0, producer=None):
        self.x, self.ldx, self.K, self.coff = x, ldx, K, coff
        self.scale, self.shift, self.relu, self.sub, self.sub_ld = scale, shift, relu, sub, sub_ld
        self.producer = producer
        self.dtype = abi.BF16 if x.dtype == torch.bfloat16 else abi.F32

    def struct(self):
        return abi.ActSrc(fptr(self.x), self.ldx, self.coff, fptr(self.scale), fptr(self.shift), int(self.relu),
                          fptr(self.sub), self.sub_ld, self.dtype)


def wgrad_rows_per_split(lib, M, K, N):
    rps, tk, tn = C.c_int(0), C.c_int(0), C.c_int(0)
    abi.check(lib.t3d_wgrad_plan(M, K, N, C.byref(rps), C.byref(tk), C.byref(tn)), 't3d_wgrad_plan')
    return rps.value


def bwd_rows_per_split(lib, M, K, N, dtype):
    rps, one = C.c_int(0), C.c_int(0)
    abi.check(lib.t3d_bwd_plan(M, K, N, dtype, C.byref(rps), C.byref(one)), 't3d_bwd_plan')
    return rps.value


def gram_rows_per_split(lib, M, K, dtype):
    rps, one = C.c_int(0), C.c_int(0)
    abi.check(lib.t3d_gram_plan(M, K, dtype, C.byref(rps), C.byref(one)), 't3d_gram_plan')
    return rps.value


class PointLayer:

    def __init__(self, g, scope, K, N, w=None, bias=None, kernel_1xD=False, w_name=None, w_row0=0, pool=False, gram=None, bn=True,
                 n_alloc=None, pooled_out=None):
        self.g, self.scope, self.K, self.N = g, scope, K, N
        self.bn = bn
        self.gram = (pool and os.environ.get('T3D_POOL_GRAM', '1') != '0') if gram is None else (gram and pool)
        self.w_name, self.w_row0 = w_name, w_row0
        rt, vs = g.rt, g.vars
        M, T = g.M, g.M // TILE
        self.M, self.T = M, T
        if w is None:
            shape = (1, K, 1, N) if kernel_1xD else (1, 1, K, N)
            fan_in, fan_out = (K, K * N) if kernel_1xD else (K, N)
            w = vs.xavier(scope + '/weights', shape, fan_in, fan_out).view(K, N)
            self.w_name = scope + '/weights'
            self.w_row0 = 0
        self.w = w
        self.dt, self.adt = g.dt, g.adt
        self.w_mm = vs.bf16_view(w) if self.dt == abi.BF16 else w
        self.w_x3, self.w_x3_d = vs.x3_frag(w, K, N) if (self.dt == abi.F32 and X3_PRESPLIT and rt.device.type == 'cuda' and rt.arith != abi.ARITH_FP32_MFMA and
                                                       getattr(vs, 'x3_frag_enabled', True)) else ((None, 0), (None, 0))
        assert not (self.dt == abi.BF16 and pool and not self.gram), "bf16: max-pooled layers take the Gram-form backward"
        self.bias = bias if bias is not None else vs.const(scope + '/biases', (N,), 0.0)
        if bn:
            self.gamma = vs.const(scope + '/bn/gamma', (N,), 1.0)
            self.beta = vs.const(scope + '/bn/beta', (N,), 0.0)
            self.mm = vs.const(scope + '/bn/moving_mean', (N,), 0.0, trainable=False)
            self.mv = vs.const(scope + '/bn/moving_variance', (N,), 1.0, trainable=False)
        self.NA = n_alloc or N
        if self.NA != N:
# ... 53 lines not shown
            f.pooled, f.ld_pooled, f.argidx, f.ysel = fptr(self.pooled), self.ld_pooled, iptr(self.argidx), fptr(self.ysel)
        plan.add('t3d_bn_fwd_finalize', f)
        self._fin_args = f
        self.out = None if self.gram else ActSpec(self.y, self.N, self.N, 0, self.scale, self.shift, True, producer=self)
        return self.out

    def enable_pool(self, rowmask=None):
        g, rt = self.g, self.g.rt
        assert self.bn and self._fin_args is not None and self.NA == self.N, 'enable_pool: a batch-normed layer with >= 64 channels'
        if not self.pool:
            T, N, B = self.T, self.N, g.B
            self.pmax, self.pmin = rt.zeros(T, N), rt.zeros(T, N)
            self.pamax, self.pamin = rt.zeros(T, N, dtype=torch.int32), rt.zeros(T, N, dtype=torch.int32)
            self.pooled, self.argidx, self.ysel = rt.zeros(B, N), rt.zeros(B, N, dtype=torch.int32), rt.zeros(B, N)
            self.ld_pooled = N
            self.pool = True
        a, f = self._fwd_args, self._fin_args
        self.rowmask = rowmask
        a.rowmask = fptr(rowmask)
        a.pmax, a.pmin, a.pamax, a.pamin = fptr(self.pmax), fptr(self.pmin), iptr(self.pamax), iptr(self.pamin)
        f.pool_pmax, f.pool_pmin, f.pool_pamax, f.pool_pamin = fptr(self.pmax), fptr(self.pmin), iptr(self.pamax), iptr(self.pamin)
        f.pool_B, f.pool_tiles_per_frustum = g.B, g.rpf // TILE
        f.pooled, f.ld_pooled, f.argidx, f.ysel = fptr(self.pooled), self.N, iptr(self.argidx), fptr(self.ysel)
        return self.pooled

    def _ensure_bwd_buffers(self):
        rt = self.g.rt
        if self.coef is None:
            self.coef = rt.zeros(3, self.N)
            if self.pool:
                self.dpool = rt.zeros(self.g.B, self.N)
                if self.gram:
                    K, N = self.K, self.N
                    self.wc, self.S = rt.zeros(N, K), rt.zeros(self.M, K)
                    self.S_live = rt.zeros(self.M, dtype=torch.int32) if SPARSE_GATED else None
                    assert self.S_live is not None or self.dt == abi.F32, "bf16: the fp32 sparse rows S need their row flags"
            else:
                self.dz = self._acquire_dz()
                self.psum_dz, self.psum_dzy = rt.zeros(self.T, self.N), rt.zeros(self.T, self.N)

    def _acquire_dz(self):
        g, rt = self.g, self.g.rt
        if not (DZ_POOL and getattr(g, 'pool_dz', True)):
            return rt.zeros(self.M, self.N, dtype=self.adt)
        pools = g.__dict__.setdefault('_dz_pools', {})
        free = pools.setdefault((self.scope.rsplit('/', 1)[0], self.adt), [])
        need = self.M * self.N
        pick = None
        for i in range(len(free) - 1, -1, -1):
            if free[i].numel() >= need:
                pick = free.pop(i)
                break
        if pick is None:
            pick = rt.zeros(need, dtype=self.adt)
        self._dz_buf = pick
        return pick[:need].view(self.M, self.N)

    def _release_dz(self):
        buf = getattr(self, '_dz_buf', None)
        if buf is not None:
            self._dz_buf = None
            self.g.__dict__.setdefault('_dz_pools', {}).setdefault((self.scope.rsplit('/', 1)[0], self.adt), []).append(buf)

    def dy_struct(self):
        if self.pool:
            return abi.DySrc(fptr(None), fptr(self.y), fptr(self.coef), iptr(self.argidx), fptr(self.dpool), self.dt)
        return abi.DySrc(fptr(self.dz), fptr(self.y), fptr(self.coef), iptr(None), fptr(None), self.dt)

    def bn_bwd(self, plan, dpool_in=None, ld_dpool_in=0, param_grads=True):
        g, vs = self.g, self.g.vars
        self._ensure_bwd_buffers()
        if self.pool and getattr(self, '_bn_bwd_fused_in', None) is plan:
# ... 54 lines not shown
        a.a, a.slabs = self.src.struct(), fptr(sl['G'])
        a.M, a.K, a.rows_per_frustum, a.rows_per_split = self.M, K, g.rpf, rps
        plan.add('t3d_pointmlp_gram', a)
        c = abi.ActColsumArgs()
        c.a, c.M, c.K, c.rows_per_frustum, c.part = self.src.struct(), self.M, K, g.rpf, fptr(sl['abar'])
        plan.add('t3d_act_colsum', c)
        if merged:
            self._emit_prep(plan, sl)
            self._gram_prepped = (plan, red)
        emit_reduce()
        f = abi.PoolWgradFinishArgs()
        f.a, f.argidx, f.dpool, f.coef = self.src.struct(), iptr(self.argidx), fptr(self.dpool), fptr(self.coef)
        f.w, f.bias, f.g, f.abar = fptr(self.w), fptr(self.bias), fptr(red['G']), fptr(red['abar'])
        f.B, f.K, f.N, f.rows_per_frustum = g.B, K, N, g.rpf
        goff = g.vars.offset(self.w_name) + self.w_row0 * N
        f.dw = fptr(g.vars.grads[goff:goff + K * N])
        plan.add('t3d_pool_wgrad_finish', f)
        self._gram_keep_w = (sl, red)

    def _dgrad_gram(self, plan):
        g, K, N = self.g, self.K, self.N
        prev = self.src.producer
        assert prev is not None and not prev.pool, 'pooled layers follow a dense per-point layer in every reference net'
        prev._ensure_bwd_buffers()
        prepped = getattr(self, '_gram_prepped', (None, None))
        if prepped[0] is plan:
            red = prepped[1]
        else:
            nch = (N + 127) // 128
            sl, red, emit_reduce = self._gram_reduce(plan, [('P', K * K, nch), ('rowconst', K, nch)])
            self._emit_prep(plan, sl)
            emit_reduce()
            self._gram_keep_d = (sl, red)
        r = abi.PoolSparseRowsArgs(iptr(self.argidx), fptr(self.dpool), fptr(self.wc), g.B, N, K, g.rpf, fptr(self.S),
                                   iptr(self.S_live))
        plan.add('t3d_pool_sparse_rows', r)
        a = abi.PointMlpDgradGramArgs()
        a.arith = self.g.rt.arith
        a.a, a.p, a.rowconst, a.add_in = self.src.struct(), fptr(red['P']), fptr(red['rowconst']), fptr(self.S)
        a.add_live = iptr(self.S_live)
        a.prev_y, a.prev_scale, a.prev_shift = fptr(prev.y), fptr(prev.scale), fptr(prev.shift)
        a.out, a.psum_dz, a.psum_dzy = fptr(prev.dz), fptr(prev.psum_dz), fptr(prev.psum_dzy)
        a.M, a.K, a.rows_per_frustum, a.dtype = self.M, K, g.rpf, self.dt
        plan.add('t3d_pointmlp_dgrad_gram', a)

    def _bwd_pair_gram(self, plan):
        g, rt, K, N = self.g, self.g.rt, self.K, self.N
        lib = rt.lib
        prev = self.src.producer
        assert prev is not None and not prev.pool
        prev._ensure_bwd_buffers()
        rps = gram_rows_per_split(lib, self.M, K, self.src.dtype)
        nch = (N + 127) // 128
        sl, red, emit_reduce = self._gram_reduce(plan, [('G', K * K, self.M // rps), ('abar', K, self.T), ('P', K * K, nch),
                                                        ('rowconst', K, nch)])
        ga = abi.PointMlpGramArgs()
        ga.arith = self.g.rt.arith
        ga.a, ga.slabs = self.src.struct(), fptr(sl['G'])
        ga.M, ga.K, ga.rows_per_frustum, ga.rows_per_split = self.M, K, g.rpf, rps
        ca = abi.ActColsumArgs()
        ca.a, ca.M, ca.K, ca.rows_per_frustum, ca.part = self.src.struct(), self.M, K, g.rpf, fptr(sl['abar'])
        qa = abi.PoolBwdPrepArgs(fptr(self.w), fptr(self.bias), fptr(self.coef), K, N, fptr(sl['P']), fptr(sl['rowconst']),
                                 fptr(self.wc))
        fn1, r1 = lib.t3d_pool_bwd_stage1, (C.byref(ga), C.byref(ca), C.byref(qa))
        plan.keep.extend([ga, ca, qa, sl, red])
        plan.calls.append(('t3d_pool_bwd_stage1', lambda s: fn1(r1[0], r1[1], r1[2], s), (ga, ca, qa)))
        plan.lanes.append(0)
        r = abi.PoolSparseRowsArgs(iptr(self.argidx), fptr(self.dpool), fptr(self.wc), g.B, N, K, g.rpf, fptr(self.S),
                                   iptr(self.S_live))
        emit_reduce(sparse=r)
        f = abi.PoolWgradFinishArgs()
        f.a, f.argidx, f.dpool, f.coef = self.src.struct(), iptr(self.argidx), fptr(self.dpool), fptr(self.coef)
        f.w, f.bias, f.g, f.abar = fptr(self.w), fptr(self.bias), fptr(red['G']), fptr(red['abar'])
        f.B, f.K, f.N, f.rows_per_frustum = g.B, K, N, g.rpf
        goff = g.vars.offset(self.w_name) + self.w_row0 * N
        f.dw = fptr(g.vars.grads[goff:goff + K * N])
        d = abi.PointMlpDgradGramArgs()
        d.arith = self.g.rt.arith
        d.a, d.p, d.rowconst, d.add_in = self.src.struct(), fptr(red['P']), fptr(red['rowconst']), fptr(self.S)
        d.add_live = iptr(self.S_live)
        d.prev_y, d.prev_scale, d.prev_shift = fptr(prev.y), fptr(prev.scale), fptr(prev.shift)
        d.out, d.psum_dz, d.psum_dzy = fptr(prev.dz), fptr(prev.psum_dz), fptr(prev.psum_dzy)
        d.M, d.K, d.rows_per_frustum, d.dtype = self.M, K, g.rpf, self.dt
        fn2, r2 = lib.t3d_pool_bwd_stage2, (C.byref(f), C.byref(d))
        plan.keep.extend([f, d])
        plan.calls.append(('t3d_pool_bwd_stage2', lambda s: fn2(r2[0], r2[1], s), (f, d)))
        plan.lanes.append(0)

    def _emit_prep(self, plan, sl):
        q = abi.PoolBwdPrepArgs(fptr(self.w), fptr(self.bias), fptr(self.coef), self.K, self.N, fptr(sl['P']),
                                fptr(sl['rowconst']), fptr(self.wc))
        plan.add('t3d_pool_bwd_prep', q)

    def wgrad(self, plan):
        with plan.side():
            self._wgrad(plan)
        self._release_dz()

    def _wgrad_args(self, fused=False):
        g = self.g
        if fused and self.src.dtype == self.dt:
            rps = bwd_rows_per_split(g.rt.lib, self.M, self.K, self.N, self.dt)
        else:
            rps = wgrad_rows_per_split(g.rt.lib, self.M, self.K, self.N)
        n_slabs = self.M // rps
        goff = g.vars.offset(self.w_name) + self.w_row0 * self.N
        soff = g.ws.reserve(goff, self.K * self.N, n_slabs)
        a = abi.PointMlpWgradArgs()
        a.arith = self.g.rt.arith
        a.a, a.dy = self.src.struct(), self.dy_struct()
        a.M, a.K, a.N, a.rows_per_frustum, a.rows_per_split = self.M, self.K, self.N, g.rpf, rps
        g.deferred_slab_ptrs.append((a, 'slabs', soff))
        return a

    def _wgrad(self, plan):
        if self.gram:
            return self._wgrad_gram(plan)
        plan.add('t3d_pointmlp_wgrad', self._wgrad_args())

    def _dgrad_args(self, out_raw=None, add_in=None):
        prev = self.src.producer if out_raw is None else None
        a = abi.PointMlpDgradArgs()
        a.arith = self.g.rt.arith
        a.dy, a.w, a.add_in, a.dtype = self.dy_struct(), fptr(self.w_mm), fptr(add_in), self.dt
# ... 151 lines not shown
```

transferable3d_amd/nets.py:

```python
import ctypes as C
import os

import numpy as np
import torch

from . import abi
from .abi import fptr, iptr
from .constants import BOX_OUT_DIMS, NUM_CLASS
from .engine import ActSpec, FcLayer, Plan, PointLayer, Runtime, VarStore, Workspace, TILE


class Graph:

    def __init__(self, batch_size, num_point, num_channel, rt=None, seed=0, unbiased_ema=True, vars=None, dtype='f32'):
        assert dtype in ('f32', 'bf16')
        self.dtype = dtype
        self.dt = abi.DTYPE_BY_NAME[dtype]
        self.adt = torch.bfloat16 if dtype == 'bf16' else torch.float32
        if num_point % TILE:
            raise abi.T3DError('num_point must be a multiple of %d' % TILE)
        self.rt = rt or Runtime()
        self.B, self.rpf, self.C = batch_size, num_point, num_channel
        self.ldpc = (num_channel + 3) // 4 * 4
        self.M = batch_size * num_point
        self.vars = vars or VarStore(self.rt, seed=seed)
        self.ws = Workspace(self.rt)
        self.unbiased_ema = unbiased_ema
        self.hyper = self.rt.zeros(4)
        self.hyper[2] = 0.5
        self.bn_decay_ptr = self.hyper[2:3]
        self.dropout_masks = {}
        self.inline_dropout, self.dropout_seed = False, 1234
        self.deferred_slab_ptrs = []
        self.dp_buckets = False
        self.buckets = []
        self.trained_prefixes = None
        self._slabs_reduced = 0
        self.fwd = Plan(self.rt)
        self.bwd = Plan(self.rt)
        self.opt = Plan(self.rt)
        self.pre = Plan(self.rt)
        self.finalized = False

    def finalize(self):
        self.ws.finalize()
        base = self.ws.buf.data_ptr()
        for a, field, soff in self.deferred_slab_ptrs:
            setattr(a, field, C.cast(C.c_void_p(base + 4 * soff), abi.F))
        self.finalized = True
        return self

    def emit_reduce_slabs(self, plan):
        ws, vs, lib = self.ws, self.vars, self.rt.lib
        plan.join()
        i0, i1 = self._slabs_reduced, len(ws.entries)
        self._slabs_reduced = i1
        if i1 == i0:
            return
        mx = max(e[2] for e in ws.entries[i0:i1])
        stride = C.sizeof(abi.SlabDesc)

        def thunk(s):
            return lib.t3d_reduce_slabs(fptr(ws.buf), fptr(vs.grads),
                                        C.cast(C.c_void_p(ws.table.data_ptr() + i0 * stride), C.POINTER(abi.SlabDesc)), i1 - i0, mx, s)
        plan.add_raw('t3d_reduce_slabs', thunk, arg={'i0': i0, 'i1': i1, 'max_numel': mx})

    def emit_cast_weights(self, plan):
        vs, lib = self.vars, self.rt.lib
        if self.dt != abi.BF16:
            from .engine import X3_PRESPLIT
            if (X3_PRESPLIT and self.rt.device.type == 'cuda' and self.rt.arith != abi.ARITH_FP32_MFMA and getattr(vs, 'x3_frag_enabled', True)
                    and hasattr(lib, 't3d_split_x3_frag')):
                def thunk(s):
                    if not getattr(vs, 'x3_frag_entries', None):
                        return 0
                    t, n, nblk = vs.frag_table()
                    pf, pd = vs.x3_frag_planes
                    return lib.t3d_split_x3_frag(fptr(vs.params), C.c_void_p(pf.data_ptr()), C.c_void_p(pd.data_ptr()), vs.x3_frag_stride,
                                                 C.c_void_p(t.data_ptr()), n, nblk, s)
                plan.add_raw('t3d_split_x3_frag', thunk, arg={'vars': vs})
            return
        p16 = vs.enable_bf16()
        plan.add_raw('t3d_cast_bf16', lambda s: lib.t3d_cast_bf16(fptr(vs.params), C.c_void_p(p16.data_ptr()), vs.used, s))

    def default_bucket(self):
        return self.vars.trainable_ranges(self.trained_prefixes)

    def declare_bucket(self, plan, prefixes):
        if not self.dp_buckets:
            return
        self.emit_reduce_slabs(plan)
        self.buckets.append(self.vars.trainable_ranges(prefixes))
        plan.bucket_ready(len(self.buckets) - 1)

    def emit_batch_assemble(self, plan, dataset, inputs, seed=0, **aug):
        equal_prob = aug.pop('equal_class_prob', 0.0)
        semi = aug.pop('semi_sampling', None)
        if semi is not None:
            slots = self.rt.zeros(self.B, dtype=torch.int32)
            plan.add('t3d_semi_sample', dataset.semi_sample_args(self.hyper, self.B, slots, inputs.is_data_2D, method=semi,
                                                                 seed=seed ^ 0x2545F491, equal_prob=equal_prob))
            if aug.pop('alternate', False):
                raise ValueError('alternate=True (the two-list walk of split_by_class) and semi_sampling=%r exclude each other' % semi)
            a = dataset.assemble_args(inputs, self.hyper, self.B, self.rpf, self.C, seed=seed, sample=slots, **aug)
            a.is_data_2D, a.frustum_is_2D, a.slot_is_2D = iptr(None), iptr(None), iptr(inputs.is_data_2D)
            plan.add('t3d_batch_assemble', a)
            return
        if equal_prob > 0.0:
            slots = self.rt.zeros(self.B, dtype=torch.int32)
            alternate = bool(aug.pop('alternate', False))
# ... 1034 lines not shown
```

transferable3d_amd/schedule.py:

```python
import ctypes as C
import os

import numpy as np
import torch

from . import abi

HOST_FN = {'t3d_pointmlp_fwd': 't3d_pointmlp_fwd_r', 't3d_pointmlp_bwd': 't3d_pointmlp_bwd_r',
           't3d_pool_bwd_stage1': 't3d_pool_bwd_stage1_r', 't3d_pool_bwd_stage2': 't3d_pool_bwd_stage2_r',
           't3d_pointmlp_wgrad': 't3d_pointmlp_wgrad_r'}
MAX_RUN = min(int(os.environ.get('T3D_RIDER_RUN', '10')), abi.RIDER_MAX_OPS)
RIDER_SLOWDOWN = float(os.environ.get('T3D_RIDER_SLOW', '1.5' if os.environ.get('T3D_X3', '1') != '0' else '1.85'))
HOST_STRETCH = float(os.environ.get('T3D_RIDER_STRETCH', '0.2'))
HOST_STRETCH_MAX = float(os.environ.get('T3D_RIDER_STRETCH_MAX', '8.0'))
RIDER_SLOT_SHARE = 16.0 / 512.0
HOST_OVERHEAD_US = float(os.environ.get('T3D_RIDER_COST', '0.5'))
RIDER_MAX_FRAC = float(os.environ.get('T3D_RIDER_MAXFRAC', '1.0'))
WIDE_SHARE = float(os.environ.get('T3D_RIDER_WIDE', '0.5'))


def _first(arg):
    return arg[0] if isinstance(arg, tuple) else arg


def is_host(lib, name, arg):
    if name not in HOST_FN or arg is None:
        return False
    fn = getattr(lib, name + '_hosts_riders', None)
    if fn is None:
        return False
    args = arg if isinstance(arg, tuple) else (arg,)
    return fn(*[C.byref(a) for a in args]) == 1


def small_op(name, arg, depends=0):
    o = abi.SmallOp()
    o.kind, o.depends = abi.RIDER_KIND[name], int(depends)
    C.memmove(C.byref(o.u), C.byref(arg), C.sizeof(arg))
    return o


def can_ride(lib, name, arg):
    if name not in abi.RIDER_KIND or arg is None or isinstance(arg, tuple) or not hasattr(lib, 't3d_riders_plan'):
        return False
    if name in abi.RIDER_WIDE and WIDE_SHARE <= 0:
        return False
    rs = abi.RiderSet()
    rs.ops[0], rs.n_ops = small_op(name, arg), 1
    return lib.t3d_riders_plan(C.byref(rs)) == 0


def can_pair(name, arg):
    if name not in abi.SMALL_KIND or arg is None:
        return False
    return not (name == 't3d_bn_bwd_finalize' and arg.psum_dz and arg.n_tiles > 512)


def _x3_requested(a):
    req = getattr(a, 'arith', abi.ARITH_AUTO) if a is not None else abi.ARITH_AUTO
    return req == abi.ARITH_BF16X3 or (req == abi.ARITH_AUTO and os.environ.get('T3D_X3', '1') != '0')


def est_us(name, arg):
    a = _first(arg) if arg is not None else None
    x3 = _x3_requested(a) and getattr(a, 'dtype', 0) == abi.F32
    if name == 't3d_pointmlp_fwd':
        if a.K <= 4:
            return 5.0
        return 6.0 + 2.0 * a.M * a.K * a.N / (float(os.environ.get('T3D_SCHED_FWD_RATE', '1.6e8')) if x3 else 1.0e8)
    if name == 't3d_pointmlp_bwd':
        return 6.0 + 4.0 * a.M * a.K * a.N / (float(os.environ.get('T3D_SCHED_BWD_RATE', '1.25e8')) if x3 else 0.95e8)
    if name == 't3d_pointmlp_wgrad':
        if a.K <= 4:
            return 7.0
        return 6.0 + 2.0 * a.M * max(a.K, 8) * a.N / 0.5e8
    if name == 't3d_pointmlp_dgrad':
        return 6.0 + 2.0 * a.M * a.K * a.N / 0.9e8
    if name == 't3d_pool_bwd_stage1':
        return 6.0 + 2.0 * a.M * a.K * a.K / 0.9e8
    if name == 't3d_pool_bwd_stage2':
        f = a
        return 8.0 + 2.0 * arg[1].M * f.K * f.K / (1.0e8 if _x3_requested(arg[1]) else 0.85e8)
    if name in ('t3d_fc_fwd', 't3d_fc_bwd', 't3d_fc_dinput'):
        rb = max(1.0, a.B / 32.0)
        kn = float(a.K) * a.N * rb
        return (8.0 + 2.5e-5 * kn) if name == 't3d_fc_bwd' else (5.5 + 1.7e-5 * kn)
    if name == 't3d_bn_fwd_finalize':
        return 6.3 if a.pool_pmax else 4.0
    if name == 't3d_pool_bwd_mid' and a is not None and hasattr(a, 'sparse'):
        return 15.0 + 1.1e-4 * a.sparse.N * a.sparse.K * max(1.0, a.sparse.B / 32.0)
    return {'t3d_bn_fwd_finalize': 4.0, 't3d_bn_bwd_finalize': 4.3, 't3d_dy_colsum': 4.0, 't3d_strong_loss': 12.0,
            't3d_pool_bwd_mid': 25.0, 't3d_small_pair': 10.0, 't3d_seg_head': 13.0, 't3d_seg_finalize': 4.0}.get(name, 6.0)


class _Op:
    __slots__ = ('call', 'name', 'arg', 'host', 'ride', 'pair', 'us', 'wide')

    def __init__(self, lib, call):
        self.call = call
        self.name, _, self.arg = call
        self.host = is_host(lib, self.name, self.arg)
        self.ride = can_ride(lib, self.name, self.arg)
        self.pair = can_pair(self.name, self.arg)
        self.us = est_us(self.name, self.arg)
        self.wide = self.name in abi.RIDER_WIDE


def align(S, T, max_run=None):
    max_run = MAX_RUN if max_run is None else max_run
    nS, nT = len(S), len(T)
    INF = float('inf')
    cost = np.full((nS + 1, nT + 1), INF)
    back = {}
    cost[0, 0] = 0.0
    chains = (S, T)

    def relax(i, j, c, step):
        if c < cost[i, j]:
            cost[i, j] = c
            back[(i, j)] = step

    for i in range(nS + 1):
# ... 59 lines not shown

    def make(self, ops):
        lib, n = self.rt.lib, len(ops)
        rs = abi.RiderSet()
        for k, (name, arg) in enumerate(ops):
            rs.ops[k] = small_op(name, arg, depends=1 if k > 0 else 0)
        rs.n_ops = n
        abi.check(lib.t3d_riders_plan(C.byref(rs)), 't3d_riders_plan')
        sync = self._row()
        rs.sync = C.cast(C.c_void_p(sync.data_ptr()), C.POINTER(C.c_uint32))
        self.sets.append((rs, None, sync, None))
        return rs

    def timeouts(self):
        n = 0
        for k, pool in enumerate(self.pools):
            rows = min(self.POOL, self.used - k * self.POOL)
            n += int((pool[:rows, self.width - 2] != 0).sum().item())
        return n

    def check(self):
        n = self.timeouts()
        if n:
            raise RiderBarrierTimeout(
                '%d rider set(s) report a barrier time-out (csrc/rider_dev.h): the small ops behind that barrier ran before their '
                'inputs were complete, so the weights / Adam moments / moving statistics written since the last check are invalid.  '
                'Restore the last checkpoint; T3D_OVERLAP=0 runs the step without riders.' % n)


def _host_call(lib, op, rs):
    fn, ref = getattr(lib, HOST_FN[op.name]), C.byref(rs)
    if isinstance(op.arg, tuple):
        refs = tuple(C.byref(a) for a in op.arg)
        if len(refs) == 2:
            thunk = lambda s, fn=fn, r=refs, ref=ref: fn(r[0], r[1], ref, s)
        else:
            thunk = lambda s, fn=fn, r=refs, ref=ref: fn(r[0], r[1], r[2], ref, s)
    else:
        aref = C.byref(op.arg)
        thunk = lambda s, fn=fn, aref=aref, ref=ref: fn(aref, ref, s)
    return (HOST_FN[op.name], thunk, op.arg)


def overlap_chains(rt, S_calls, T_calls, sets, max_run=None):
    lib = rt.lib
    S = [_Op(lib, c) for c in S_calls]
    T = [_Op(lib, c) for c in T_calls]
    steps, total = align(S, T, max_run)
    chains = (S, T)
    out, rep = [], {'serial_us': sum(o.us for o in S + T), 'scheduled_us': total, 'hosted': 0, 'rider_ops': 0, 'pairs': 0, 'solo': 0,
                    'lines': []}
    short = lambda o: '%s%s[%.0f]' % ('ST'[o in T and o not in S], o.name[4:], o.us)
    for st in steps:
        if st[0] == 'solo':
            out.append(chains[st[1]][st[2]].call)
            rep['solo'] += 1
            rep['lines'].append(short(chains[st[1]][st[2]]))
        elif st[0] == 'host':
            _, ch, p, q0, q1 = st
            riders = chains[1 - ch][q0:q1]
            rs = sets.make([(o.name, o.arg) for o in riders])
            out.append(_host_call(lib, chains[ch][p], rs))
            rep['hosted'] += 1
            rep['rider_ops'] += len(riders)
            rep['lines'].append('%s  <- %s' % (short(chains[ch][p]), ' , '.join(short(o) for o in riders)))
        else:
            _, i, j = st
# ... 11 lines not shown
```

transferable3d_amd/step.py:

```python
import ctypes as C
import os

import numpy as np
import torch

from . import abi
from .abi import fptr
from .engine import Plan


OPTIMIZER_CALLS = ('t3d_adam_tf_step', 't3d_momentum_step')


class TrainStep:
    def __init__(self, engine, pre, fwd, bwd=None, opt=None, process_group=None, use_hip_graph=None, force_dist=False,
                 one_graph=None, fuse_head_tail=None):
        self.e, self.rt = engine, engine.rt
        if fuse_head_tail is None:
            fuse_head_tail = os.environ.get('T3D_FUSE_HEAD_TAIL', '1') != '0'
        self.fuse_head_tail = bool(fuse_head_tail)
        self.fused = []
        self.pre, self.fwd, self.bwd, self.opt = pre, fwd, bwd, opt
        self.train = bwd is not None
        self.pg = process_group
# ... 80 lines not shown
            merged.two_streams = two
            for kind, x in tail:
                if kind == 'run':
                    merged.calls.extend(x.calls)
                    merged.lanes.extend(x.lanes)
            prog = prog[:k] + [t for t in tail if t[0] == 'wait'] + [('run', merged)]
        return prog

    def _fuse_head_tail(self, calls, lanes):
        lib, e = self.rt.lib, self.e
        self.fused = []
        real = [i for i, c in enumerate(calls) if not c[0].startswith('__') or c[0] in (Plan.BUCKET, Plan.WAIT, Plan.FLUSH)]
        names = [calls[i][0] for i in real]
        drop = set()

        def adjacent(*want):
            for k in range(len(names) - len(want) + 1):
                if tuple(names[k:k + len(want)]) == want:
                    idx = real[k:k + len(want)]
                    if all(calls[i][2] is not None for i in idx) and not any(lanes[i] for i in idx):
                        return idx
            return None

        idx = adjacent('t3d_schedule_step', 't3d_split_x3_frag', 't3d_pointmlp_fwd')
        if idx is not None and self.on_gpu and hasattr(lib, 't3d_step_head') and self.rt.arith == abi.ARITH_BF16X3 and \
                names.count('t3d_schedule_step') == 1:
            sc, vs, a = calls[idx[0]][2], calls[idx[1]][2]['vars'], calls[idx[2]][2]
            if lib.t3d_step_head_takes(C.byref(a)) == 1 and getattr(vs, 'x3_frag_entries', None):
                hyper, sched = sc['hyper'], sc['sched']

                def head(s, a=a, vs=vs, hyper=hyper, sched=sched):
                    t, n, nblk = vs.frag_table()
                    pf, pd = vs.x3_frag_planes
                    return lib.t3d_step_head(C.byref(a), fptr(vs.params), C.c_void_p(pf.data_ptr()), C.c_void_p(pd.data_ptr()),
                                             vs.x3_frag_stride, C.c_void_p(t.data_ptr()), n, nblk, fptr(hyper), C.byref(sched), s)
                calls[idx[0]] = ('t3d_step_head', head, None)
                drop.update(idx[1:])
                self.fused.append('t3d_step_head')
        idx = adjacent('t3d_reduce_slabs', 't3d_adam_tf_step')
        vs = e.vars
        if idx is not None and self.on_gpu and hasattr(lib, 't3d_reduce_slabs_adam') and not self.dist and e.dt == abi.F32 and \
                names.count('t3d_adam_tf_step') == 1 and idx[1] == real[-1] and getattr(e, 'trained_prefixes', None) is None:
            rd, ad = calls[idx[0]][2], calls[idx[1]][2]
            if (ad['off'], ad['n']) == (0, vs.used) and e.finalized:
                ws = e.ws
                ent = ws.entries[rd['i0']:rd['i1']]
                ranges, nblk = abi.adam_range_table(vs.used, [(go, ne) for _, go, ne, _ in ent])
                host = (abi.AdamRange * max(len(ranges), 1))()
                for i, (off, n, blk0) in enumerate(ranges):
                    host[i] = abi.AdamRange(off, n, blk0, 0)
                table = torch.as_tensor(np.frombuffer(bytes(host), dtype=np.uint8).copy()).to(self.rt.device)
                stride = C.sizeof(abi.SlabDesc)

                def tail(s, rd=rd, ad=ad, table=table, n_ranges=len(ranges), nblk=nblk):
                    return lib.t3d_reduce_slabs_adam(
                        fptr(ws.buf), fptr(vs.grads), C.cast(C.c_void_p(ws.table.data_ptr() + rd['i0'] * stride), C.POINTER(abi.SlabDesc)),
                        rd['i1'] - rd['i0'], rd['max_numel'], fptr(vs.params), fptr(vs.adam_m), fptr(vs.adam_v),
                        C.cast(C.c_void_p(table.data_ptr()), C.POINTER(abi.AdamRange)), n_ranges, nblk, fptr(e.hyper),
                        ad['beta1'], ad['beta2'], ad['eps'], ad['grad_scale'], s)
                calls[idx[0]] = ('t3d_reduce_slabs_adam', tail, None)
                drop.add(idx[1])
                self.fused.append('t3d_reduce_slabs_adam')
        keep = [i for i in range(len(calls)) if i not in drop]
        return [calls[i] for i in keep], [lanes[i] for i in keep]

    def _overlap(self, calls, lanes):
# ... 174 lines not shown

    def n_launches(self):
        return sum(len(p) for p in ([self.pre] if self.pre is not None else []) + [self.fwd] + ([self.bwd, self.opt] if self.train else []))

    def n_graph_segments(self, generate_masks=True):
        ent = self.cache.get(bool(generate_masks))
        if ent is None or ent['graphs'] is None:
            return 0
        return len(ent['graphs'])


WORKLOADS = ('A', 'boxpc', 'F')


def workload_flags(workload):
    from .config import make_parser
    if workload == 'A':
        c = make_parser().parse_special_args(['--SEMI_MODEL', 'A', '--WEAK_WEIGHT_REPROJECTION', '0', '--WEAK_WEIGHT_SURFACE', '0'])
        import os
        c.WEAK_LOSS_SUMMARIES = os.environ.get('T3D_WEAK_SUMMARIES', '0') == '1'
        return c
    if workload == 'boxpc':
        return make_parser().parse_special_args(['--BOX_PC_MASK_REPRESENTATION', 'A', '--BOXPC_WEIGHT_DELTA', '4'])
    return make_parser().parse_special_args(
        ['--SEMI_MODEL', 'F', '--BOX_PC_MASK_REPRESENTATION', 'A', '--WEAK_WEIGHT_INTRACLASSVAR', '2', '--WEAK_WEIGHT_REPROJECTION', '0',
         '--SEMI_MULTIPLIER_FOR_WEAK_LOSS', '0.05', '--SEMI_BOXPC_FIT_ONLY_ON_2D_CLS', '1', '--SEMI_WEIGHT_BOXPC_FIT_LOSS', '1'])


STAGE_C_TRAIN_CLASSES = [i in (1, 2, 6, 7, 8) for i in range(10)]


def build_training_step(rt, workload, B, N, C, world=1, rank=0, process_group=None, force_dist=False, flat_allreduce=False,
                        use_hip_graph=None, inline_dropout=True, dropout_seed=1234, seed=0, state_dict=None, c=None, dtype='f32',
                        one_graph=None, fuse_head_tail=None):
    from .nets import BoxPCModel, Graph, SemiModelA, SemiModelF, make_schedule
    assert workload in WORKLOADS
    g = Graph(B, N, C, rt=rt, seed=seed, dtype=dtype)
    g.inline_dropout, g.dropout_seed = inline_dropout, dropout_seed + rank
    c = c if c is not None else workload_flags(workload)
    prefixes = None
    if workload == 'A':
        model = SemiModelA(g, c)
        loss = model.loss_op.loss
    elif workload == 'boxpc':
        model = BoxPCModel(g, c, False)
        loss = model.loss_op.loss
    else:
        model = SemiModelF(g, c, use_one_hot=True, train_classes=STAGE_C_TRAIN_CLASSES)
        loss = model.loss
        prefixes = list(SemiModelF.VAR_LIST)
    if state_dict is not None:
        g.vars.load_state_dict(state_dict)
    dist_on = process_group is not None and (world > 1 or force_dist)
    g.dp_buckets = dist_on and not flat_allreduce
    g.emit_schedule(g.pre, make_schedule(B * world))
    g.emit_dropout_masks(g.pre, seed=dropout_seed + rank)
    if workload == 'F':
        model.emit_forward(g.fwd, True, True, train=True)
    else:
        model.emit_forward(g.fwd, True, True)
    model.emit_backward(g.bwd)
    g.emit_adam(g.opt, prefixes=prefixes, grad_scale=1.0 / world)
    g.finalize()
    step = TrainStep(g, g.pre, g.fwd, g.bwd, g.opt, process_group=process_group, use_hip_graph=use_hip_graph,
                     force_dist=force_dist, one_graph=one_graph, fuse_head_tail=fuse_head_tail)
    return g, model, step, loss


class _Program:

    def __init__(self, rt, calls, want_graph):
# ... 126 lines not shown
```

Measured before the change: 27520.

## Fold pool sparse-rows into backward stage1 using pre-transposed weights

Moves the pool sparse-rows computation out of the mid reduction kernel into the stage1 pool backward launch as extra workgroups. Instead of depending on the wc buffer produced by prep in the same stage, the new path reads a transposed copy of the weights. That copy is built by extra blocks added to the split_x3_frag and step_head kernels. The mid reduce kernel then only does the slab reduction, which shortens the critical path between stage1 and stage2. The cost is more complexity, an extra weight-transpose buffer kept in sync each step, and more work packed into stage1.

Measured after the change: 27640, median of 6. No clear change (+0.4%).

```diff
diff --git a/include/t3d.h b/include/t3d.h
--- a/include/t3d.h
+++ b/include/t3d.h
@@ -215,6 +215,18 @@
 int t3d_pool_sparse_rows(const t3d_pool_sparse_rows_args* args, t3d_stream_t stream);
 
 typedef struct {
+  const int32_t* argidx;
+  const float* dpool;
+  const float* wt;
+  const float* coef;
+  int B, N, K;
+  int rows_per_frustum;
+  float* s;
+  int32_t* row_live;
+} t3d_pool_sparse_rows_wt_args;
+int t3d_pool_sparse_rows_wt(const t3d_pool_sparse_rows_wt_args* args, t3d_stream_t stream);
+
+typedef struct {
   uint32_t struct_size;
   t3d_act_src a;
   const float* p;
@@ -274,6 +286,8 @@
                         const t3d_pool_bwd_prep_args* prep, t3d_stream_t stream);
 int t3d_pool_bwd_stage2(const t3d_pool_wgrad_finish_args* finish, const t3d_pointmlp_dgrad_gram_args* dgrad,
                         t3d_stream_t stream);
+int t3d_pool_bwd_stage1_takes_sparse(const t3d_pointmlp_gram_args* gram, const t3d_act_colsum_args* colsum,
+                                     const t3d_pool_bwd_prep_args* prep, const t3d_pool_sparse_rows_wt_args* sparse);
 
 typedef struct {
   const float* in;  int ld_in;  int K;
@@ -750,6 +764,19 @@
                   const t3d_x3_frag_entry* table, int n_entries, int n_blocks, float* hyper, const t3d_schedule* sched,
                   t3d_stream_t stream);
 
+typedef struct {
+  int64_t off;
+  float* wt;
+  int32_t K, N;
+  int32_t blk0;
+  int32_t reserved;
+} t3d_wt_entry;
+int t3d_split_x3_frag_wt(const float* params, void* planes_fwd, void* planes_dgrad, int64_t plane_stride, const t3d_x3_frag_entry* table,
+                         int n_entries, int n_blocks, const t3d_wt_entry* wt_table, int n_wt, int n_wt_blocks, t3d_stream_t stream);
+int t3d_step_head_wt(const t3d_pointmlp_fwd_args* fwd, const float* params, void* planes_fwd, void* planes_dgrad, int64_t plane_stride,
+                     const t3d_x3_frag_entry* table, int n_entries, int n_blocks, float* hyper, const t3d_schedule* sched,
+                     const t3d_wt_entry* wt_table, int n_wt, int n_wt_blocks, t3d_stream_t stream);
+
 int t3d_momentum_step(float* params, const float* grads, float* accum, int64_t n, const float* hyper, float momentum,
                       float grad_scale, t3d_stream_t stream);
 
@@ -810,6 +837,8 @@
                           const t3d_rider_set* riders, t3d_stream_t stream);
 int t3d_pool_bwd_stage2_r(const t3d_pool_wgrad_finish_args* finish, const t3d_pointmlp_dgrad_gram_args* dgrad,
                           const t3d_rider_set* riders, t3d_stream_t stream);
+int t3d_pool_bwd_stage1_sr(const t3d_pointmlp_gram_args* gram, const t3d_act_colsum_args* colsum, const t3d_pool_bwd_prep_args* prep,
+                           const t3d_pool_sparse_rows_wt_args* sparse, const t3d_rider_set* riders, t3d_stream_t stream);
 int t3d_pointmlp_fwd_hosts_riders(const t3d_pointmlp_fwd_args* args);
 int t3d_pointmlp_wgrad_hosts_riders(const t3d_pointmlp_wgrad_args* args);
 int t3d_pointmlp_bwd_hosts_riders(const t3d_pointmlp_dgrad_args* dgrad, const t3d_pointmlp_wgrad_args* wgrad);
diff --git a/transferable3d_amd/abi.py b/transferable3d_amd/abi.py
--- a/transferable3d_amd/abi.py
+++ b/transferable3d_amd/abi.py
@@ -74,6 +74,11 @@
                 ('row_live', I)]
 
 
+class PoolSparseRowsWtArgs(C.Structure):
+    _fields_ = [('argidx', I), ('dpool', F), ('wt', F), ('coef', F), ('B', i32), ('N', i32), ('K', i32), ('rows_per_frustum', i32), ('s', F),
+                ('row_live', I)]
+
+
 class PointMlpDgradGramArgs(Sized):
     _fields_ = [('struct_size', C.c_uint32), ('a', ActSrc), ('p', F), ('rowconst', F), ('add_in', F), ('add_live', I), ('prev_y', F), ('prev_scale', F),
                 ('prev_shift', F),
@@ -230,6 +235,20 @@
     for i, (off, K, N) in enumerate(entries):
         rec[i] = (off, K, N, 1, 1, blk, 0)
         blk += (K * N // 8 + 255) // 256
+    return rec.view(np.uint8).copy(), blk
+
+
+class WtEntry(C.Structure):
+    _fields_ = [('off', C.c_int64), ('wt', F), ('K', C.c_int32), ('N', C.c_int32), ('blk0', C.c_int32), ('reserved', C.c_int32)]
+
+
+def wt_table(entries):
+    import numpy as np
+    rec = np.zeros(len(entries), dtype=np.dtype([('off', '<i8'), ('wt', '<u8'), ('K', '<i4'), ('N', '<i4'), ('blk0', '<i4'), ('reserved', '<i4')]))
+    blk = 0
+    for i, (off, wt, K, N) in enumerate(entries):
+        rec[i] = (off, wt, K, N, blk, 0)
+        blk += ((K + 31) // 32) * ((N + 31) // 32)
     return rec.view(np.uint8).copy(), blk
 
 
@@ -481,6 +500,11 @@
     't3d_dy_colsum': [C.POINTER(DyColsumArgs), VP],
     't3d_pool_bwd_prep': [C.POINTER(PoolBwdPrepArgs), VP],
     't3d_pool_sparse_rows': [C.POINTER(PoolSparseRowsArgs), VP],
+    't3d_pool_sparse_rows_wt': [C.POINTER(PoolSparseRowsWtArgs), VP],
+    't3d_pool_bwd_stage1_sr': [C.POINTER(PointMlpGramArgs), C.POINTER(ActColsumArgs), C.POINTER(PoolBwdPrepArgs), C.POINTER(PoolSparseRowsWtArgs),
+                               C.POINTER(RiderSet), VP],
+    't3d_pool_bwd_stage1_takes_sparse': [C.POINTER(PointMlpGramArgs), C.POINTER(ActColsumArgs), C.POINTER(PoolBwdPrepArgs),
+                                         C.POINTER(PoolSparseRowsWtArgs)],
     't3d_pointmlp_dgrad_gram': [C.POINTER(PointMlpDgradGramArgs), VP],
     't3d_pointmlp_gram': [C.POINTER(PointMlpGramArgs), VP],
     't3d_act_colsum': [C.POINTER(ActColsumArgs), VP],
@@ -516,6 +540,8 @@
     't3d_reduce_slabs_adam': [F, F, C.POINTER(SlabDesc), i32, i32, F, F, F, C.POINTER(AdamRange), i32, i32, F, f32, f32, f32, f32, VP],
     't3d_step_head_takes': [C.POINTER(PointMlpFwdArgs)],
     't3d_step_head': [C.POINTER(PointMlpFwdArgs), F, VP, VP, C.c_int64, VP, i32, i32, F, C.POINTER(Schedule), VP],
+    't3d_step_head_wt': [C.POINTER(PointMlpFwdArgs), F, VP, VP, C.c_int64, VP, i32, i32, F, C.POINTER(Schedule), VP, i32, i32, VP],
+    't3d_split_x3_frag_wt': [F, VP, VP, C.c_int64, VP, i32, i32, VP, i32, i32, VP],
     't3d_adam_tf_step': [F, F, F, F, C.c_int64, F, f32, f32, f32, f32, VP],
     't3d_momentum_step': [F, F, F, C.c_int64, F, f32, f32, VP],
     't3d_split_x3': [F, VP, C.c_int64, C.c_int64, VP],
diff --git a/transferable3d_amd/csrc/bn_optim.hip b/transferable3d_amd/csrc/bn_optim.hip
--- a/transferable3d_amd/csrc/bn_optim.hip
+++ b/transferable3d_amd/csrc/bn_optim.hip
@@ -281,12 +281,18 @@
 extern "C" int t3d_pool_bwd_mid(const float* slab_base, float* grad_base, const t3d_slab_desc* table_dev, int n_tensors,
                                 int max_numel, const t3d_pool_sparse_rows_args* a, t3d_stream_t stream) {
   if (!slab_base || !grad_base || !table_dev || n_tensors <= 0) return T3D_ERR_ARG;
-  const int rc = check_sparse_rows(a);
-  if (rc != T3D_OK) return rc;
   int gx = (max_numel / 4 + 31) / 32;
   if (gx > 256) gx = 256;
   if (gx < 1) gx = 1;
   const int n_reduce = gx * n_tensors;
+  if (!a || !a->argidx) {
+    T3D_LAUNCH(k_pool_bwd_mid, dim3(n_reduce), dim3(256), 8 * 32 * sizeof(float4), static_cast<hipStream_t>(stream), slab_base, grad_base,
+               table_dev, gx, n_reduce, t3d_pool_sparse_rows_args{});
+    T3D_CHECK_LAUNCH();
+    return T3D_OK;
+  }
+  const int rc = check_sparse_rows(a);
+  if (rc != T3D_OK) return rc;
   const long M = (long)a->B * a->rows_per_frustum;
   const int n_sparse = (int)(M / 128) * (a->K / SR_KC);
   const size_t lds = sparse_rows_lds(a->N);
diff --git a/transferable3d_amd/csrc/pointmlp.hip b/transferable3d_amd/csrc/pointmlp.hip
--- a/transferable3d_amd/csrc/pointmlp.hip
+++ b/transferable3d_amd/csrc/pointmlp.hip
@@ -2886,6 +2886,54 @@
   }
 }
 
+template <int GT, class PR>
+__global__ __launch_bounds__(NT, MIN_WAVES_PER_EU) void k_pool_bwd_stage1_s(const t3d_pointmlp_gram_args g, const t3d_act_colsum_args c,
+                                                                     const t3d_pool_bwd_prep_args q, const int n_gram,
+                                                                     const int n_colsum, const t3d_pool_sparse_rows_wt_args sp,
+                                                                     const int n_sparse) {
+  extern __shared__ __attribute__((aligned(16))) float smem[];
+  if ((int)blockIdx.x < n_sparse) {
+    const int tiles = n_sparse / (sp.K / SR_KC);
+    pool_sparse_rows_wt_body(sp, smem, (int)blockIdx.x % tiles, (int)blockIdx.x / tiles);
+    return;
+  }
+  const int b = blockIdx.x - n_sparse;
+  if (b < n_gram) {
+    typename PR::template Act<false, typename PR::T> la{g.a, g.K, g.rows_per_frustum};
+    wgrad_body<GT, GT, PR, true>(la, la, g.slabs, g.K, g.K, g.rows_per_split, smem, b, n_gram);
+  } else if (b < n_gram + n_colsum) {
+    act_colsum_body<typename PR::T>(c, smem, b - n_gram);
+  } else {
+    const int r = b - n_gram - n_colsum, kb = q.K / 32;
+    pool_bwd_prep_body(q, smem, r % kb, (r / kb) % kb, r / (kb * kb));
+  }
+}
+
+template <int GT, class PR>
+__global__ __launch_bounds__(NT, MIN_WAVES_PER_EU) void k_pool_bwd_stage1_rs(const t3d_pointmlp_gram_args g, const t3d_act_colsum_args c,
+                                                                      const t3d_pool_bwd_prep_args q, const int n_gram,
+                                                                      const int n_colsum, const t3d_pool_sparse_rows_wt_args sp,
+                                                                      const int n_sparse, const t3d_rider_set r) {
+  extern __shared__ __attribute__((aligned(16))) float smem[];
+  if ((int)blockIdx.x < r.n_wg) { run_riders(r, smem); return; }
+  const int bs = blockIdx.x - r.n_wg;
+  if (bs < n_sparse) {
+    const int tiles = n_sparse / (sp.K / SR_KC);
+    pool_sparse_rows_wt_body(sp, smem, bs % tiles, bs / tiles);
+    return;
+  }
+  const int b = bs - n_sparse;
+  if (b < n_gram) {
+    typename PR::template Act<false, float> la{g.a, g.K, g.rows_per_frustum};
+    wgrad_body<GT, GT, PR, true>(la, la, g.slabs, g.K, g.K, g.rows_per_split, smem, b, n_gram);
+  } else if (b < n_gram + n_colsum) {
+    act_colsum_body<float>(c, smem, b - n_gram);
+  } else {
+    const int rr = b - n_gram - n_colsum, kb = q.K / 32;
+    pool_bwd_prep_body(q, smem, rr % kb, (rr / kb) % kb, rr / (kb * kb));
+  }
+}
+
 template <int BN, class PR = PathF32>
 __global__ __launch_bounds__(NT, MIN_WAVES_PER_EU) void k_pool_bwd_stage2_r(const t3d_pool_wgrad_finish_args f,
                                                                      const t3d_pointmlp_dgrad_gram_args d, const int n_finish,
@@ -3489,13 +3537,16 @@
 int t3d_x3_bwd(const t3d_pointmlp_dgrad_args* d, const t3d_pointmlp_wgrad_args* w, const t3d_rider_set* r, int tk, int tn, bool wide,
                int n_w, int n_d, hipStream_t s);
 int t3d_x3_stage1(const t3d_pointmlp_gram_args* g, const t3d_act_colsum_args* c, const t3d_pool_bwd_prep_args* q, const t3d_rider_set* r,
-                  int gt, int n_gram, int n_colsum, int n_prep, size_t lds_other, hipStream_t s);
+                  int gt, int n_gram, int n_colsum, int n_prep, size_t lds_other, const t3d_pool_sparse_rows_wt_args* sp, int n_sparse,
+                  hipStream_t s);
 int t3d_x3_stage2(const t3d_pool_wgrad_finish_args* f, const t3d_pointmlp_dgrad_gram_args* d, const t3d_rider_set* r, bool wide,
                   int n_finish, int n_d, size_t lds_other, hipStream_t s);
 int t3d_x3_split(const float* src, void* planes, int64_t n, int64_t plane_stride, hipStream_t s);
-int t3d_x3_split_frag(const float* params, void* pf, void* pd, int64_t stride, const t3d_x3_frag_entry* tab, int n, int n_blocks, hipStream_t s);
+int t3d_x3_split_frag(const float* params, void* pf, void* pd, int64_t stride, const t3d_x3_frag_entry* tab, int n, int n_blocks,
+                      const t3d_wt_entry* wtab, int n_wt, int n_wt_blocks, hipStream_t s);
 int t3d_x3_step_head(const t3d_pointmlp_fwd_args* a, const float* params, void* pf, void* pd, int64_t stride, const t3d_x3_frag_entry* tab, int n,
-                     int n_blocks, float* hyper, const t3d_schedule* sched, hipStream_t s);
+                     int n_blocks, float* hyper, const t3d_schedule* sched, const t3d_wt_entry* wtab, int n_wt, int n_wt_blocks,
+                     hipStream_t s);
 int t3d_x3_dgrad(const t3d_pointmlp_dgrad_args* a, bool wide, hipStream_t s);
 int t3d_x3_wgrad(const t3d_pointmlp_wgrad_args* a, int tk, int tn, int n_blocks, hipStream_t s);
 int t3d_x3_gram(const t3d_pointmlp_gram_args* a, int tk, int n_blocks, hipStream_t s);
@@ -3567,35 +3618,66 @@
     *reinterpret_cast<bf16x8*>(d + 2 * stride) = __builtin_shufflevector(l0, l1, 0, 1, 2, 3, 4, 5, 6, 7);
   }
 }
+__device__ __forceinline__ void wt_transpose_body(const float* __restrict__ params, const t3d_wt_entry* __restrict__ tab,
+                                                  int n, const int blk) {
+  __shared__ float t[32][33];
+  int e = 0;
+  while (e + 1 < n && blk >= tab[e + 1].blk0) ++e;
+  const t3d_wt_entry en = tab[e];
+  const int tn = (en.N + 31) / 32, r = blk - en.blk0;
+  const int k0 = (r / tn) * 32, n0 = (r % tn) * 32;
+  if (k0 >= en.K) return;
+  const float* w = params + en.off;
+  float* o = en.wt;
+  const int x = threadIdx.x & 31, y = threadIdx.x >> 5;
+#pragma unroll
+  for (int q = 0; q < 4; ++q) {
+    const int k = k0 + y + 8 * q, c = n0 + x;
+    if (k < en.K && c < en.N) t[y + 8 * q][x] = w[(long)k * en.N + c];
+  }
+  __syncthreads();
+#pragma unroll
+  for (int q = 0; q < 4; ++q) {
+    const int c = n0 + y + 8 * q, k = k0 + x;
+    if (c < en.N && k < en.K) o[(long)c * en.K + k] = t[x][y + 8 * q];
+  }
+}
 __global__ __launch_bounds__(256) void k_split_x3_frag(const float* __restrict__ params, bf16_t* __restrict__ pf, bf16_t* __restrict__ pd, long stride,
-                                                       const t3d_x3_frag_entry* __restrict__ tab, int n) {
-  split_x3_frag_body(params, pf, pd, stride, tab, n, (int)blockIdx.x);
+                                                       const t3d_x3_frag_entry* __restrict__ tab, int n, const int n_split,
+                                                       const t3d_wt_entry* __restrict__ wtab, const int n_wt) {
+  if ((int)blockIdx.x < n_split) split_x3_frag_body(params, pf, pd, stride, tab, n, (int)blockIdx.x);
+  else wt_transpose_body(params, wtab, n_wt, (int)blockIdx.x - n_split);
 }
 
 template <int N>
 __global__ __launch_bounds__(NT) void k_step_head(const t3d_pointmlp_fwd_args p, const int n_fwd, const float* __restrict__ params,
                                                   bf16_t* __restrict__ pf, bf16_t* __restrict__ pd, const long stride,
                                                   const t3d_x3_frag_entry* __restrict__ tab, const int n, const int n_split, float* hyper,
-                                                  const t3d_schedule sched) {
+                                                  const t3d_schedule sched, const t3d_wt_entry* __restrict__ wtab,
+                                                  const int n_wt, const int n_wt_blocks) {
   __shared__ float red[2][NT / (N / 8)][N];
   const int b = blockIdx.x;
   if (b < n_fwd) pointmlp_fwd_tinyk_body<N, float>(p, red, b);
   else if (b < n_fwd + n_split) split_x3_frag_body(params, pf, pd, stride, tab, n, b - n_fwd);
+  else if (b < n_fwd + n_split + n_wt_blocks) wt_transpose_body(params, wtab, n_wt, b - n_fwd - n_split);
   else if (threadIdx.x < 64) schedule_step_body(hyper, sched, threadIdx.x);
 }
 }
 int t3d_x3_step_head(const t3d_pointmlp_fwd_args* a, const float* params, void* pf, void* pd, int64_t stride, const t3d_x3_frag_entry* tab, int n,
-                     int n_blocks, float* hyper, const t3d_schedule* sched, hipStream_t s) {
-  static_assert(NT == 256, "the three roles of k_step_head are 256-thread workgroups");
+                     int n_blocks, float* hyper, const t3d_schedule* sched, const t3d_wt_entry* wtab, int n_wt, int n_wt_blocks,
+                     hipStream_t s) {
+  static_assert(NT == 256, "the roles of k_step_head are 256-thread workgroups");
   const int n_fwd = a->M / 128;
-  const dim3 grid(n_fwd + n_blocks + 1);
-  if (a->N == 64) T3D_LAUNCH(k_step_head<64>, grid, dim3(NT), 0, s, *a, n_fwd, params, static_cast<bf16_t*>(pf), static_cast<bf16_t*>(pd), (long)stride, tab, n, n_blocks, hyper, *sched);
-  else T3D_LAUNCH(k_step_head<128>, grid, dim3(NT), 0, s, *a, n_fwd, params, static_cast<bf16_t*>(pf), static_cast<bf16_t*>(pd), (long)stride, tab, n, n_blocks, hyper, *sched);
+  const dim3 grid(n_fwd + n_blocks + n_wt_blocks + 1);
+  if (a->N == 64) T3D_LAUNCH(k_step_head<64>, grid, dim3(NT), 0, s, *a, n_fwd, params, static_cast<bf16_t*>(pf), static_cast<bf16_t*>(pd), (long)stride, tab, n, n_blocks, hyper, *sched, wtab, n_wt, n_wt_blocks);
+  else T3D_LAUNCH(k_step_head<128>, grid, dim3(NT), 0, s, *a, n_fwd, params, static_cast<bf16_t*>(pf), static_cast<bf16_t*>(pd), (long)stride, tab, n, n_blocks, hyper, *sched, wtab, n_wt, n_wt_blocks);
   T3D_CHECK_LAUNCH();
   return T3D_OK;
 }
-int t3d_x3_split_frag(const float* params, void* pf, void* pd, int64_t stride, const t3d_x3_frag_entry* tab, int n, int n_blocks, hipStream_t s) {
-  T3D_LAUNCH(k_split_x3_frag, dim3(n_blocks), dim3(256), 0, s, params, static_cast<bf16_t*>(pf), static_cast<bf16_t*>(pd), (long)stride, tab, n);
+int t3d_x3_split_frag(const float* params, void* pf, void* pd, int64_t stride, const t3d_x3_frag_entry* tab, int n, int n_blocks,
+                      const t3d_wt_entry* wtab, int n_wt, int n_wt_blocks, hipStream_t s) {
+  T3D_LAUNCH(k_split_x3_frag, dim3(n_blocks + n_wt_blocks), dim3(256), 0, s, params, static_cast<bf16_t*>(pf), static_cast<bf16_t*>(pd), (long)stride, tab, n,
+             n_blocks, wtab, n_wt);
   T3D_CHECK_LAUNCH();
   return T3D_OK;
 }
@@ -3727,7 +3809,24 @@
 }
 
 int t3d_x3_stage1(const t3d_pointmlp_gram_args* g, const t3d_act_colsum_args* c, const t3d_pool_bwd_prep_args* q, const t3d_rider_set* r,
-                  int gt, int n_gram, int n_colsum, int n_prep, size_t lds_other, hipStream_t s) {
+                  int gt, int n_gram, int n_colsum, int n_prep, size_t lds_other, const t3d_pool_sparse_rows_wt_args* sp, int n_sparse,
+                  hipStream_t s) {
+  if (gt != 64) return T3D_ERR_ARG;
+  if (sp) {
+    const dim3 grid_s(n_sparse + n_gram + n_colsum + n_prep + (r ? r->n_wg : 0));
+    const size_t lds_s = lds_with(lds_max(lds_max(lds_wgrad_x3(gt, gt), lds_other), sparse_rows_wt_lds(sp->N)), r);
+    if (r) {
+      auto kern = k_pool_bwd_stage1_rs<64, PathX3>;
+      allow_lds(reinterpret_cast<const void*>(kern), lds_s);
+      T3D_LAUNCH(kern, grid_s, dim3(NT), lds_s, s, *g, *c, *q, n_gram, n_colsum, *sp, n_sparse, *r);
+    } else {
+      auto kern = k_pool_bwd_stage1_s<64, PathX3>;
+      allow_lds(reinterpret_cast<const void*>(kern), lds_s);
+      T3D_LAUNCH(kern, grid_s, dim3(NT), lds_s, s, *g, *c, *q, n_gram, n_colsum, *sp, n_sparse);
+    }
+    T3D_CHECK_LAUNCH();
+    return T3D_OK;
+  }
   const dim3 grid(n_gram + n_colsum + n_prep + (r ? r->n_wg : 0));
   const size_t lds = lds_with(lds_max(lds_wgrad_x3(gt, gt), lds_other), r);
 #define T3D_ST1X(GT_)                                                                  \
@@ -4310,6 +4409,24 @@
   return T3D_OK;
 }
 
+static bool stage1_takes_sparse(const t3d_pointmlp_gram_args* g, const t3d_act_colsum_args* c, const t3d_pool_sparse_rows_wt_args* sp) {
+  static const bool on = []() { const char* e = getenv("T3D_STAGE1_SPARSE"); return !(e && e[0] == '0'); }();
+  if (!on || g->a.dtype == T3D_BF16 || c->a.dtype != g->a.dtype || gram1_ok(g) || !x3_layer_bwd(g->arith, g->K, g->K)) return false;
+  return (long)sp->B * sp->rows_per_frustum == g->M && sp->K == g->K && sp->rows_per_frustum == g->rows_per_frustum &&
+         sparse_rows_wt_lds(sp->N) <= 76 * 1024;
+}
+
+extern "C" int t3d_pool_bwd_stage1_takes_sparse(const t3d_pointmlp_gram_args* g, const t3d_act_colsum_args* c, const t3d_pool_bwd_prep_args* q,
+                                                const t3d_pool_sparse_rows_wt_args* sp) {
+  T3D_ABI_TAKE(pointmlp_gram_args, g);
+  int rc = check_gram(g);
+  if (rc != T3D_OK) return rc;
+  if ((rc = check_colsum(c)) != T3D_OK) return rc;
+  if ((rc = check_prep(q)) != T3D_OK) return rc;
+  if ((rc = check_sparse_rows_wt(sp)) != T3D_OK) return rc;
+  return stage1_takes_sparse(g, c, sp) ? 1 : 0;
+}
+
 extern "C" int t3d_pool_bwd_stage1(const t3d_pointmlp_gram_args* g, const t3d_act_colsum_args* c,
                                    const t3d_pool_bwd_prep_args* q, t3d_stream_t stream) {
   return t3d_pool_bwd_stage1_r(g, c, q, nullptr, stream);
@@ -4317,6 +4434,11 @@
 
 extern "C" int t3d_pool_bwd_stage1_r(const t3d_pointmlp_gram_args* g, const t3d_act_colsum_args* c,
                                      const t3d_pool_bwd_prep_args* q, const t3d_rider_set* r, t3d_stream_t stream) {
+  return t3d_pool_bwd_stage1_sr(g, c, q, nullptr, r, stream);
+}
+
+extern "C" int t3d_pool_bwd_stage1_sr(const t3d_pointmlp_gram_args* g, const t3d_act_colsum_args* c, const t3d_pool_bwd_prep_args* q,
+                                      const t3d_pool_sparse_rows_wt_args* sp, const t3d_rider_set* r, t3d_stream_t stream) {
   T3D_ABI_TAKE(pointmlp_gram_args, g);
   if (r && !riders_ok(r)) return T3D_ERR_ARG;
   int rc = check_gram(g);
@@ -4325,6 +4447,11 @@
   if ((rc = check_prep(q)) != T3D_OK) return rc;
   hipStream_t s = static_cast<hipStream_t>(stream);
   if (c->a.dtype != g->a.dtype) return T3D_ERR_ARG;
+  if (sp) {
+    if ((rc = check_sparse_rows_wt(sp)) != T3D_OK) return rc;
+    if (!stage1_takes_sparse(g, c, sp)) return T3D_ERR_ARG;
+  }
+  const int n_sparse = sp ? (int)(((long)sp->B * sp->rows_per_frustum) / 128) * (sp->K / SR_KC) : 0;
   if (gram1_ok(g) && c->M == g->M && c->K == g->K && c->a.x == g->a.x && c->a.ldx == g->a.ldx && c->a.coff == g->a.coff) {
     T3D_RIDERS_FIRST(r, stream);
     const int n_gram1 = g->M / g->rows_per_split, n_prep1 = (q->K / 32) * (q->K / 32) * ((q->N + PCH - 1) / PCH);
@@ -4354,7 +4481,7 @@
   if (PREP_LDS > lds) lds = PREP_LDS;
   if (COLSUM_LDS > lds) lds = COLSUM_LDS;
   T3D_HOSTED(r, stream);
-  if (x3g) return t3d_x3_stage1(g, c, q, r, gt, n_gram, n_colsum, n_prep, lds_max(PREP_LDS, COLSUM_LDS), s);
+  if (x3g) return t3d_x3_stage1(g, c, q, r, gt, n_gram, n_colsum, n_prep, lds_max(PREP_LDS, COLSUM_LDS), sp, n_sparse, s);
   lds = lds_with(lds, r);
 #define T3D_ST1(GT_, PR_)                                                              \
   do {                                                                                 \
@@ -4453,7 +4580,23 @@
   if (!params || !planes_fwd || !planes_dgrad || !table || n_entries <= 0 || n_blocks <= 0 || plane_stride <= 0 || (plane_stride & 7) ||
       (reinterpret_cast<uintptr_t>(params) & 15) || (reinterpret_cast<uintptr_t>(planes_fwd) & 15) || (reinterpret_cast<uintptr_t>(planes_dgrad) & 15))
     return T3D_ERR_ARG;
-  return t3d_x3_split_frag(params, planes_fwd, planes_dgrad, plane_stride, table, n_entries, n_blocks, static_cast<hipStream_t>(stream));
+  return t3d_x3_split_frag(params, planes_fwd, planes_dgrad, plane_stride, table, n_entries, n_blocks, nullptr, 0, 0, static_cast<hipStream_t>(stream));
+}
+
+static bool wt_args_ok(const t3d_wt_entry* wt_table, int n_wt, int n_wt_blocks) {
+  if (n_wt == 0) return n_wt_blocks == 0;
+  return wt_table != nullptr && n_wt > 0 && n_wt_blocks > 0 && n_wt_blocks <= (1 << 20);
+}
+
+extern "C" int t3d_split_x3_frag_wt(const float* params, void* planes_fwd, void* planes_dgrad, int64_t plane_stride, const t3d_x3_frag_entry* table,
+                                    int n_entries, int n_blocks, const t3d_wt_entry* wt_table, int n_wt, int n_wt_blocks,
+                                    t3d_stream_t stream) {
+  if (!params || !planes_fwd || !planes_dgrad || !table || n_entries <= 0 || n_blocks <= 0 || plane_stride <= 0 || (plane_stride & 7) ||
+      (reinterpret_cast<uintptr_t>(params) & 15) || (reinterpret_cast<uintptr_t>(planes_fwd) & 15) || (reinterpret_cast<uintptr_t>(planes_dgrad) & 15) ||
+      !wt_args_ok(wt_table, n_wt, n_wt_blocks))
+    return T3D_ERR_ARG;
+  return t3d_x3_split_frag(params, planes_fwd, planes_dgrad, plane_stride, table, n_entries, n_blocks, wt_table, n_wt, n_wt_blocks,
+                           static_cast<hipStream_t>(stream));
 }
 
 static int step_head_fwd_check(const t3d_pointmlp_fwd_args* a) {
@@ -4473,14 +4616,22 @@
 extern "C" int t3d_step_head(const t3d_pointmlp_fwd_args* a, const float* params, void* planes_fwd, void* planes_dgrad, int64_t plane_stride,
                              const t3d_x3_frag_entry* table, int n_entries, int n_blocks, float* hyper, const t3d_schedule* sched,
                              t3d_stream_t stream) {
+  return t3d_step_head_wt(a, params, planes_fwd, planes_dgrad, plane_stride, table, n_entries, n_blocks, hyper, sched, nullptr, 0, 0, stream);
+}
+
+extern "C" int t3d_step_head_wt(const t3d_pointmlp_fwd_args* a, const float* params, void* planes_fwd, void* planes_dgrad, int64_t plane_stride,
+                                const t3d_x3_frag_entry* table, int n_entries, int n_blocks, float* hyper, const t3d_schedule* sched,
+                                const t3d_wt_entry* wt_table, int n_wt, int n_wt_blocks, t3d_stream_t stream) {
   T3D_ABI_TAKE(pointmlp_fwd_args, a);
+  if (!wt_args_ok(wt_table, n_wt, n_wt_blocks)) return T3D_ERR_ARG;
   if (!hyper || !sched) return T3D_ERR_ARG;
   if (!params || !planes_fwd || !planes_dgrad || !table || n_entries <= 0 || n_blocks <= 0 || plane_stride <= 0 || (plane_stride & 7) ||
       (reinterpret_cast<uintptr_t>(params) & 15) || (reinterpret_cast<uintptr_t>(planes_fwd) & 15) || (reinterpret_cast<uintptr_t>(planes_dgrad) & 15))
     return T3D_ERR_ARG;
   const int rc = step_head_fwd_check(a);
   if (rc != T3D_OK) return rc;
-  return t3d_x3_step_head(a, params, planes_fwd, planes_dgrad, plane_stride, table, n_entries, n_blocks, hyper, sched, static_cast<hipStream_t>(stream));
+  return t3d_x3_step_head(a, params, planes_fwd, planes_dgrad, plane_stride, table, n_entries, n_blocks, hyper, sched, wt_table, n_wt, n_wt_blocks,
+                          static_cast<hipStream_t>(stream));
 }
 
 static const t3d_rider_set* query_set() {
diff --git a/transferable3d_amd/csrc/poolbwd.hip b/transferable3d_amd/csrc/poolbwd.hip
--- a/transferable3d_amd/csrc/poolbwd.hip
+++ b/transferable3d_amd/csrc/poolbwd.hip
@@ -9,6 +9,10 @@
 __global__ __launch_bounds__(256) void k_pool_sparse_rows(const t3d_pool_sparse_rows_args p) {
   extern __shared__ __attribute__((aligned(16))) float smem[];
   pool_sparse_rows_body(p, smem, blockIdx.x, blockIdx.y);
+}
+__global__ __launch_bounds__(256) void k_pool_sparse_rows_wt(const t3d_pool_sparse_rows_wt_args p) {
+  extern __shared__ __attribute__((aligned(16))) float smem[];
+  pool_sparse_rows_wt_body(p, smem, blockIdx.x, blockIdx.y);
 }
 template <class XT>
 __global__ __launch_bounds__(256) void k_act_colsum(const t3d_act_colsum_args p) {
@@ -48,6 +52,21 @@
   return T3D_OK;
 }
 
+extern "C" int t3d_pool_sparse_rows_wt(const t3d_pool_sparse_rows_wt_args* a, t3d_stream_t stream) {
+  const int rc = check_sparse_rows_wt(a);
+  if (rc != T3D_OK) return rc;
+  const size_t lds = sparse_rows_wt_lds(a->N);
+  static size_t allowed = 0;
+  if (lds > 64 * 1024 && lds > allowed) {
+    (void)hipFuncSetAttribute(reinterpret_cast<const void*>(k_pool_sparse_rows_wt), hipFuncAttributeMaxDynamicSharedMemorySize, (int)lds);
+    allowed = lds;
+  }
+  const long M = (long)a->B * a->rows_per_frustum;
+  T3D_LAUNCH(k_pool_sparse_rows_wt, dim3(M / 128, a->K / SR_KC), dim3(256), lds, static_cast<hipStream_t>(stream), *a);
+  T3D_CHECK_LAUNCH();
+  return T3D_OK;
+}
+
 extern "C" int t3d_act_colsum(const t3d_act_colsum_args* a, t3d_stream_t stream) {
   const int rc = check_colsum(a);
   if (rc != T3D_OK) return rc;
diff --git a/transferable3d_amd/csrc/poolbwd_dev.h b/transferable3d_amd/csrc/poolbwd_dev.h
--- a/transferable3d_amd/csrc/poolbwd_dev.h
+++ b/transferable3d_amd/csrc/poolbwd_dev.h
@@ -124,6 +124,74 @@
       float2 cur = *t;
       cur.x = fmaf(g[u], wv[u].x, cur.x);
       cur.y = fmaf(g[u], wv[u].y, cur.y);
+      *t = cur;
+    }
+  }
+  __syncthreads();
+  const bool gated = p.row_live != nullptr;
+  if (gated && by == 0 && tid < 128) p.row_live[row0 + tid] = hitrow[tid];
+  for (int f = tid; f < 128 * SR_KC / 4; f += 256) {
+    const int r = f / (SR_KC / 4), c4 = f % (SR_KC / 4);
+    if (gated && !hitrow[r]) continue;
+    *reinterpret_cast<float4*>(p.s + (size_t)(row0 + r) * p.K + kc0 + 4 * c4) = reinterpret_cast<const float4*>(tile)[f];
+  }
+}
+
+__device__ __forceinline__ void pool_sparse_rows_wt_body(const t3d_pool_sparse_rows_wt_args& p, float* smem, int bx, int by) {
+  float* tile = smem;
+  unsigned short* lists = reinterpret_cast<unsigned short*>(smem + 128 * SR_KC);
+  int* hitrow = reinterpret_cast<int*>(lists + 4 * p.N);
+  const int tid = threadIdx.x, lane = tid & 63, w = tid >> 6;
+  const int row0 = bx * 128, kc0 = by * SR_KC;
+  const int b = row0 / p.rows_per_frustum, rin0 = row0 - b * p.rows_per_frustum;
+  for (int f = tid; f < 128 * SR_KC / 4; f += 256) reinterpret_cast<float4*>(tile)[f] = make_float4(0.f, 0.f, 0.f, 0.f);
+  if (tid < 128) hitrow[tid] = 0;
+  unsigned short* mine = lists + w * p.N;
+  int cnt = 0;
+  for (int nb = 0; nb < p.N; nb += 64 * SR_PRE) {
+    int rr[SR_PRE];
+#pragma unroll
+    for (int q = 0; q < SR_PRE; ++q) {
+      const int n = nb + 64 * q + lane;
+      rr[q] = p.argidx[(size_t)b * p.N + min(n, p.N - 1)];
+    }
+#pragma unroll
+    for (int q = 0; q < SR_PRE; ++q) {
+      const int n = nb + 64 * q + lane;
+      const int r = rr[q] - rin0;
+      const bool hit = n < p.N && r >= 0 && r < 128 && (r & 3) == w;
+      const unsigned long long m = __ballot(hit);
+      if (hit) mine[cnt + __popcll(m & ((1ull << lane) - 1ull))] = (unsigned short)n;
+      cnt += __popcll(m);
+    }
+  }
+  __syncthreads();
+  for (int i0 = 0; i0 < cnt; i0 += SR_UNROLL) {
+    float2 wv[SR_UNROLL];
+    float g[SR_UNROLL], c0[SR_UNROLL];
+    int rr[SR_UNROLL], en[SR_UNROLL];
+#pragma unroll
+    for (int u = 0; u < SR_UNROLL; ++u) en[u] = mine[min(i0 + u, cnt - 1)];
+#pragma unroll
+    for (int u = 0; u < SR_UNROLL; ++u) {
+      const int n = en[u];
+      rr[u] = p.argidx[(size_t)b * p.N + n];
+      g[u] = p.dpool[(size_t)b * p.N + n];
+      c0[u] = p.coef[n];
+      wv[u] = *reinterpret_cast<const float2*>(p.wt + (size_t)n * p.K + kc0 + 2 * lane);
+    }
+#pragma unroll
+    for (int u = 0; u < SR_UNROLL; ++u) {
+      rr[u] = (rr[u] - rin0) & 127;
+      hitrow[rr[u]] = 1;
+      g[u] = (i0 + u < cnt) ? g[u] : 0.f;
+    }
+#pragma unroll
+    for (int u = 0; u < SR_UNROLL; ++u) {
+      float2* t = reinterpret_cast<float2*>(tile + rr[u] * SR_KC + 2 * lane);
+      float2 cur = *t;
+      cur.x = fmaf(g[u], __fmul_rn(c0[u], wv[u].x), cur.x);
+      cur.y = fmaf(g[u], __fmul_rn(c0[u], wv[u].y), cur.y);
       *t = cur;
     }
   }
@@ -275,6 +343,14 @@
     return T3D_ERR_SHAPE;
   return T3D_OK;
 }
+inline size_t sparse_rows_wt_lds(int N) { return (size_t)128 * SR_KC * sizeof(float) + (size_t)4 * N * sizeof(unsigned short) + 128 * sizeof(int); }
+inline int check_sparse_rows_wt(const t3d_pool_sparse_rows_wt_args* a) {
+  if (!a || !a->argidx || !a->dpool || !a->wt || !a->coef || !a->s) return T3D_ERR_ARG;
+  if (a->B <= 0 || a->N <= 0 || a->N > 65535 || a->N % 4 || a->K <= 0 || a->K % SR_KC || a->rows_per_frustum <= 0 ||
+      a->rows_per_frustum % T3D_TILE_ROWS || sparse_rows_wt_lds(a->N) > 160 * 1024)
+    return T3D_ERR_SHAPE;
+  return T3D_OK;
+}
 inline int check_colsum(const t3d_act_colsum_args* a) {
   if (!a || !a->part || !pool_act_ok(a->a, a->K)) return T3D_ERR_ARG;
   if (a->M <= 0 || a->M % T3D_TILE_ROWS || (a->K != 64 && a->K != 128 && a->K != 256) || a->a.ldx % 4 || a->a.coff % 4)
diff --git a/transferable3d_amd/csrc/rider_dev.h b/transferable3d_amd/csrc/rider_dev.h
--- a/transferable3d_amd/csrc/rider_dev.h
+++ b/transferable3d_amd/csrc/rider_dev.h
@@ -48,6 +48,7 @@
   return gx > 256 ? 256 : (gx < 1 ? 1 : gx);
 }
 __host__ __device__ __forceinline__ int mid_sparse_blocks(const t3d_pool_sparse_rows_args& sp) {
+  if (sp.argidx == nullptr) return 0;
   return (int)(((long)sp.B * sp.rows_per_frustum) / 128) * (sp.K / SR_KC);
 }
 
@@ -116,7 +117,9 @@
     case T3D_SMALL_DY_COLSUM: return (o.u.dy_colsum.B * o.u.dy_colsum.N + 255) / 256;
     case T3D_SMALL_POOL_BWD_MID: {
       const t3d_pool_bwd_mid_args& m = o.u.mid;
-      if (!m.slab_base || !m.grad_base || !m.table_dev || m.n_tensors <= 0 || check_sparse_rows(&m.sparse) != T3D_OK) return -1;
+      if (!m.slab_base || !m.grad_base || !m.table_dev || m.n_tensors <= 0) return -1;
+      if (m.sparse.argidx == nullptr) return mid_gx(m.max_numel) * m.n_tensors;
+      if (check_sparse_rows(&m.sparse) != T3D_OK) return -1;
       if (sparse_rows_lds(m.sparse.N) > 76 * 1024) return -1;
       return mid_gx(m.max_numel) * m.n_tensors + mid_sparse_blocks(m.sparse);
     }
@@ -125,7 +128,7 @@
 }
 
 inline size_t rider_op_lds(const t3d_small_op& o) {
-  if (o.kind == T3D_SMALL_POOL_BWD_MID) return sparse_rows_lds(o.u.mid.sparse.N);
+  if (o.kind == T3D_SMALL_POOL_BWD_MID && o.u.mid.sparse.argidx != nullptr) return sparse_rows_lds(o.u.mid.sparse.N);
   return fc_lds_bytes(32);
 }
 
diff --git a/transferable3d_amd/engine.py b/transferable3d_amd/engine.py
--- a/transferable3d_amd/engine.py
+++ b/transferable3d_amd/engine.py
@@ -238,6 +238,28 @@
             self.x3_frag_table = (torch.from_numpy(raw).to(self.rt.device), len(ent), blocks)
         return self.x3_frag_table
 
+    def wt_register(self, w, K, N):
+        off = (w.data_ptr() - self.params.data_ptr()) // 4
+        lib = self.rt.lib
+        if (getattr(self, 'x3_frag_planes', None) is None or not hasattr(lib, 't3d_split_x3_frag_wt') or not hasattr(lib, 't3d_step_head_wt') or
+                not (0 <= off and off + w.numel() <= self.params.numel() and w.is_contiguous()) or w.numel() != K * N):
+            return None
+        ent = self.__dict__.setdefault('wt_entries', {})
+        if off not in ent:
+            ent[off] = (K, N, self.rt.zeros(N, K))
+            self._wt_table = None
+        assert ent[off][:2] == (K, N)
+        return ent[off][2]
+
+    def wt_table(self):
+        ent = getattr(self, 'wt_entries', None)
+        if not ent:
+            return None
+        if getattr(self, '_wt_table', None) is None:
+            raw, blocks = abi.wt_table([(off, t.data_ptr(), K, N) for off, (K, N, t) in sorted(ent.items())])
+            self._wt_table = (torch.from_numpy(raw).to(self.rt.device), len(ent), blocks)
+        return self._wt_table
+
     def bf16_view(self, w):
         off = (w.data_ptr() - self.params.data_ptr()) // 4
         assert 0 <= off and off + w.numel() <= self.params.numel() and w.is_contiguous()
@@ -348,6 +370,14 @@
     rps, one = C.c_int(0), C.c_int(0)
     abi.check(lib.t3d_gram_plan(M, K, dtype, C.byref(rps), C.byref(one)), 't3d_gram_plan')
     return rps.value
+
+
+class Stage1Args(tuple):
+
+    def __new__(cls, args, sparse):
+        self = super().__new__(cls, args)
+        self.sparse = sparse
+        return self
 
 
 class PointLayer:
@@ -467,12 +497,17 @@
                 self.dpool = rt.zeros(self.g.B, self.N)
                 if self.gram:
                     K, N = self.K, self.N
-                    self.wc, self.S = rt.zeros(N, K), rt.zeros(self.M, K)
+                    self.wc, self.S = None, rt.zeros(self.M, K)
                     self.S_live = rt.zeros(self.M, dtype=torch.int32) if SPARSE_GATED else None
                     assert self.S_live is not None or self.dt == abi.F32, "bf16: the fp32 sparse rows S need their row flags"
             else:
                 self.dz = self._acquire_dz()
                 self.psum_dz, self.psum_dzy = rt.zeros(self.T, self.N), rt.zeros(self.T, self.N)
+
+    def _wc_buf(self):
+        if self.wc is None:
+            self.wc = self.g.rt.zeros(self.N, self.K)
+        return self.wc
 
     def _acquire_dz(self):
         g, rt = self.g, self.g.rt
@@ -593,7 +628,7 @@
             self._emit_prep(plan, sl)
             emit_reduce()
             self._gram_keep_d = (sl, red)
-        r = abi.PoolSparseRowsArgs(iptr(self.argidx), fptr(self.dpool), fptr(self.wc), g.B, N, K, g.rpf, fptr(self.S),
+        r = abi.PoolSparseRowsArgs(iptr(self.argidx), fptr(self.dpool), fptr(self._wc_buf()), g.B, N, K, g.rpf, fptr(self.S),
                                    iptr(self.S_live))
         plan.add('t3d_pool_sparse_rows', r)
         a = abi.PointMlpDgradGramArgs()
@@ -621,15 +656,25 @@
         ga.M, ga.K, ga.rows_per_frustum, ga.rows_per_split = self.M, K, g.rpf, rps
         ca = abi.ActColsumArgs()
         ca.a, ca.M, ca.K, ca.rows_per_frustum, ca.part = self.src.struct(), self.M, K, g.rpf, fptr(sl['abar'])
-        qa = abi.PoolBwdPrepArgs(fptr(self.w), fptr(self.bias), fptr(self.coef), K, N, fptr(sl['P']), fptr(sl['rowconst']),
-                                 fptr(self.wc))
-        fn1, r1 = lib.t3d_pool_bwd_stage1, (C.byref(ga), C.byref(ca), C.byref(qa))
+        qa = abi.PoolBwdPrepArgs(fptr(self.w), fptr(self.bias), fptr(self.coef), K, N, fptr(sl['P']), fptr(sl['rowconst']), fptr(None))
+        sp = self._stage1_sparse(ga, ca, qa)
+        r1 = (C.byref(ga), C.byref(ca), C.byref(qa))
         plan.keep.extend([ga, ca, qa, sl, red])
-        plan.calls.append(('t3d_pool_bwd_stage1', lambda s: fn1(r1[0], r1[1], r1[2], s), (ga, ca, qa)))
+        if sp is not None:
+            fns, rsp = lib.t3d_pool_bwd_stage1_sr, C.byref(sp)
+            plan.keep.append(sp)
+            plan.calls.append(('t3d_pool_bwd_stage1', lambda s: fns(r1[0], r1[1], r1[2], rsp, None, s), Stage1Args((ga, ca, qa), sp)))
+        else:
+            qa.wc = fptr(self._wc_buf())
+            fn1 = lib.t3d_pool_bwd_stage1
+            plan.calls.append(('t3d_pool_bwd_stage1', lambda s: fn1(r1[0], r1[1], r1[2], s), (ga, ca, qa)))
         plan.lanes.append(0)
-        r = abi.PoolSparseRowsArgs(iptr(self.argidx), fptr(self.dpool), fptr(self.wc), g.B, N, K, g.rpf, fptr(self.S),
-                                   iptr(self.S_live))
-        emit_reduce(sparse=r)
+        if sp is not None:
+            emit_reduce(sparse=abi.PoolSparseRowsArgs())
+        else:
+            r = abi.PoolSparseRowsArgs(iptr(self.argidx), fptr(self.dpool), fptr(self._wc_buf()), g.B, N, K, g.rpf, fptr(self.S),
+                                       iptr(self.S_live))
+            emit_reduce(sparse=r)
         f = abi.PoolWgradFinishArgs()
         f.a, f.argidx, f.dpool, f.coef = self.src.struct(), iptr(self.argidx), fptr(self.dpool), fptr(self.coef)
         f.w, f.bias, f.g, f.abar = fptr(self.w), fptr(self.bias), fptr(red['G']), fptr(red['abar'])
@@ -648,9 +693,25 @@
         plan.calls.append(('t3d_pool_bwd_stage2', lambda s: fn2(r2[0], r2[1], s), (f, d)))
         plan.lanes.append(0)
 
+    def _stage1_sparse(self, ga, ca, qa):
+        g, rt, lib = self.g, self.g.rt, self.g.rt.lib
+        planes = (self.dt == abi.F32 and X3_PRESPLIT and rt.device.type == 'cuda' and rt.arith != abi.ARITH_FP32_MFMA and
+                  getattr(g.vars, 'x3_frag_enabled', True) and hasattr(lib, 't3d_split_x3_frag'))
+        if not getattr(g, 'stage1_sparse', False) or not planes or not hasattr(lib, 't3d_pool_bwd_stage1_takes_sparse'):
+            return None
+        sp = abi.PoolSparseRowsWtArgs(iptr(self.argidx), fptr(self.dpool), fptr(self.w), fptr(self.coef), g.B, self.N, self.K, g.rpf,
+                                      fptr(self.S), iptr(self.S_live))
+        if lib.t3d_pool_bwd_stage1_takes_sparse(C.byref(ga), C.byref(ca), C.byref(qa), C.byref(sp)) != 1:
+            return None
+        wt = g.vars.wt_register(self.w, self.K, self.N)
+        if wt is None:
+            return None
+        sp.wt = fptr(wt)
+        return sp
+
     def _emit_prep(self, plan, sl):
         q = abi.PoolBwdPrepArgs(fptr(self.w), fptr(self.bias), fptr(self.coef), self.K, self.N, fptr(sl['P']),
-                                fptr(sl['rowconst']), fptr(self.wc))
+                                fptr(sl['rowconst']), fptr(self._wc_buf()))
         plan.add('t3d_pool_bwd_prep', q)
 
     def wgrad(self, plan):
diff --git a/transferable3d_amd/nets.py b/transferable3d_amd/nets.py
--- a/transferable3d_amd/nets.py
+++ b/transferable3d_amd/nets.py
@@ -33,6 +33,7 @@
         self.inline_dropout, self.dropout_seed = False, 1234
         self.deferred_slab_ptrs = []
         self.dp_buckets = False
+        self.stage1_sparse = os.environ.get('T3D_STAGE1_SPARSE', '1') != '0'
         self.buckets = []
         self.trained_prefixes = None
         self._slabs_reduced = 0
@@ -76,6 +77,10 @@
                         return 0
                     t, n, nblk = vs.frag_table()
                     pf, pd = vs.x3_frag_planes
+                    wt = vs.wt_table()
+                    if wt is not None:
+                        return lib.t3d_split_x3_frag_wt(fptr(vs.params), C.c_void_p(pf.data_ptr()), C.c_void_p(pd.data_ptr()), vs.x3_frag_stride,
+                                                        C.c_void_p(t.data_ptr()), n, nblk, C.c_void_p(wt[0].data_ptr()), wt[1], wt[2], s)
                     return lib.t3d_split_x3_frag(fptr(vs.params), C.c_void_p(pf.data_ptr()), C.c_void_p(pd.data_ptr()), vs.x3_frag_stride,
                                                  C.c_void_p(t.data_ptr()), n, nblk, s)
                 plan.add_raw('t3d_split_x3_frag', thunk, arg={'vars': vs})
diff --git a/transferable3d_amd/schedule.py b/transferable3d_amd/schedule.py
--- a/transferable3d_amd/schedule.py
+++ b/transferable3d_amd/schedule.py
@@ -16,6 +16,8 @@
 RIDER_SLOT_SHARE = 16.0 / 512.0
 HOST_OVERHEAD_US = float(os.environ.get('T3D_RIDER_COST', '0.5'))
 RIDER_MAX_FRAC = float(os.environ.get('T3D_RIDER_MAXFRAC', '1.0'))
+STAGE1_SPARSE_US_PER_NK = 0.85e-4
+MID_REDUCE_US = 4.0
 WIDE_SHARE = float(os.environ.get('T3D_RIDER_WIDE', '0.5'))
 
 
@@ -77,7 +79,10 @@
     if name == 't3d_pointmlp_dgrad':
         return 6.0 + 2.0 * a.M * a.K * a.N / 0.9e8
     if name == 't3d_pool_bwd_stage1':
-        return 6.0 + 2.0 * a.M * a.K * a.K / 0.9e8
+        us = 6.0 + 2.0 * a.M * a.K * a.K / 0.9e8
+        if getattr(arg, 'sparse', None) is not None:
+            us += STAGE1_SPARSE_US_PER_NK * arg.sparse.N * arg.sparse.K * max(1.0, arg.sparse.B / 32.0)
+        return us
     if name == 't3d_pool_bwd_stage2':
         f = a
         return 8.0 + 2.0 * arg[1].M * f.K * f.K / (1.0e8 if _x3_requested(arg[1]) else 0.85e8)
@@ -88,6 +93,8 @@
     if name == 't3d_bn_fwd_finalize':
         return 6.3 if a.pool_pmax else 4.0
     if name == 't3d_pool_bwd_mid' and a is not None and hasattr(a, 'sparse'):
+        if not a.sparse.argidx:
+            return MID_REDUCE_US
         return 15.0 + 1.1e-4 * a.sparse.N * a.sparse.K * max(1.0, a.sparse.B / 32.0)
     return {'t3d_bn_fwd_finalize': 4.0, 't3d_bn_bwd_finalize': 4.3, 't3d_dy_colsum': 4.0, 't3d_strong_loss': 12.0,
             't3d_pool_bwd_mid': 25.0, 't3d_small_pair': 10.0, 't3d_seg_head': 13.0, 't3d_seg_finalize': 4.0}.get(name, 6.0)
@@ -213,7 +220,11 @@
     fn, ref = getattr(lib, HOST_FN[op.name]), C.byref(rs)
     if isinstance(op.arg, tuple):
         refs = tuple(C.byref(a) for a in op.arg)
-        if len(refs) == 2:
+        sp = getattr(op.arg, 'sparse', None)
+        if sp is not None:
+            fn, rsp = lib.t3d_pool_bwd_stage1_sr, C.byref(sp)
+            thunk = lambda s, fn=fn, r=refs, rsp=rsp, ref=ref: fn(r[0], r[1], r[2], rsp, ref, s)
+        elif len(refs) == 2:
             thunk = lambda s, fn=fn, r=refs, ref=ref: fn(r[0], r[1], ref, s)
         else:
             thunk = lambda s, fn=fn, r=refs, ref=ref: fn(r[0], r[1], r[2], ref, s)
diff --git a/transferable3d_amd/step.py b/transferable3d_amd/step.py
--- a/transferable3d_amd/step.py
+++ b/transferable3d_amd/step.py
@@ -136,6 +136,11 @@
                 def head(s, a=a, vs=vs, hyper=hyper, sched=sched):
                     t, n, nblk = vs.frag_table()
                     pf, pd = vs.x3_frag_planes
+                    wt = vs.wt_table()
+                    if wt is not None:
+                        return lib.t3d_step_head_wt(C.byref(a), fptr(vs.params), C.c_void_p(pf.data_ptr()), C.c_void_p(pd.data_ptr()),
+                                                    vs.x3_frag_stride, C.c_void_p(t.data_ptr()), n, nblk, fptr(hyper), C.byref(sched),
+                                                    C.c_void_p(wt[0].data_ptr()), wt[1], wt[2], s)
                     return lib.t3d_step_head(C.byref(a), fptr(vs.params), C.c_void_p(pf.data_ptr()), C.c_void_p(pd.data_ptr()),
                                              vs.x3_frag_stride, C.c_void_p(t.data_ptr()), n, nblk, fptr(hyper), C.byref(sched), s)
                 calls[idx[0]] = ('t3d_step_head', head, None)
@@ -376,11 +381,13 @@
 
 def build_training_step(rt, workload, B, N, C, world=1, rank=0, process_group=None, force_dist=False, flat_allreduce=False,
                         use_hip_graph=None, inline_dropout=True, dropout_seed=1234, seed=0, state_dict=None, c=None, dtype='f32',
-                        one_graph=None, fuse_head_tail=None):
+                        one_graph=None, fuse_head_tail=None, stage1_sparse=None):
     from .nets import BoxPCModel, Graph, SemiModelA, SemiModelF, make_schedule
     assert workload in WORKLOADS
     g = Graph(B, N, C, rt=rt, seed=seed, dtype=dtype)
     g.inline_dropout, g.dropout_seed = inline_dropout, dropout_seed + rank
+    if stage1_sparse is not None:
+        g.stage1_sparse = bool(stage1_sparse)
     c = c if c is not None else workload_flags(workload)
     prefixes = None
     if workload == 'A':
```
